# tonyckc/WT-PSE-code

Measured on AMD Instinct MI355X. Metric: training images/sec (256x256 fundus) — full WT-PSE iteration, higher is better.
Workload: dtype f32 (layers with > 16 output channels and the fused 1x1 heads: x2h (2 fp16 terms per fp32 operand — power-of-two operand scaling —, 3 fp16 MFMA products per multiply, fp32 accumulation); the 16-channel layers the same on 16x16x32, the 1-/3-channel input layers and small 1x1 convs fp32-input MFMA)

## Files before the change

### include/wtpse_hip.h

```cpp
#ifndef WTPSE_HIP_H
#define WTPSE_HIP_H
#ifdef __cplusplus
extern "C" {
#endif


int wtpse_pack_conv_weights(const float* params, const int* desc, int n_desc, float* packed, void* stream);

int wtpse_conv_fwd(const float* in0, int C0, const float* in1, int C1, const float* wpacked, const float* bias,
                   const float* pro0, const float* pro1, int pro_relu, float* out0, float* out1, int Csplit, float* stats,
                   int B, int H, int W, int Cout, int ksize, int relu_out, const float* mask_ref, unsigned* out_amax, void* stream);
int wtpse_conv_stats_blocks(int B, int H, int W);
int wtpse_conv_fwd_gram(const float* in0, int C0, const float* wpacked, const float* bias, const float* pro0, int pro_relu,
                        float* out0, float* gram_partial, int B, int H, int W, int Cout, int relu_out, unsigned* out_amax,
                        void* stream);

int wtpse_conv_x3_stats_blocks(int B, int H, int W, int Cout, int ksize);
int wtpse_x3r_enable(int on);
int wtpse_x3_xcd(int on);
int wtpse_x3_small_wide(int on);
int wtpse_x3_terms(int terms);
int wtpse_amax(const float* x, long long n, unsigned* amax_table, void* stream);
int wtpse_pack_conv_weights_x3(const float* params, const int* desc, int n_desc, unsigned short* packed, void* stream);
int wtpse_conv_fwd_x3(const float* in0, int C0, const float* in1, int C1, const unsigned short* wpacked, const float* bias,
                      const float* pro0, const float* pro1, int pro_relu, float* out0, float* out1, int Csplit, float* stats,
                      int B, int H, int W, int Cout, int ksize, int relu_out, const float* mask_ref, const unsigned* in_amax,
                      const unsigned* in_amax1, unsigned* out_amax, void* stream);

int wtpse_conv16_x3(const float* in0, int C0, const unsigned short* wx16, const float* bias, const float* pro0, int pro_relu,
                    float* out0, float* stats, float* gram_partial, const float* mask_ref, const float* bn_ss,
                    const float* bn_mean, int bn_relu, int B, int H, int W, int Cout, int relu_out, int in_is_grad,
                    const unsigned* in_amax, unsigned* out_amax, void* stream);
int wtpse_pack_conv16_x3(const float* params, const int* desc, int n_desc, unsigned short* packed, void* stream);

int wtpse_dgrad_bnb(const float* dy, int C, const float* wpacked, float* out0, float* out1, int Csplit, const float* bn_y,
                    const float* bn_ss, const float* bn_mean, int bn_relu, int bn_c0, int bn_c1, float* stats, int B, int H, int W,
                    int Cout, int ksize, void* stream);
int wtpse_dgrad_x3_bnb(const float* dy, int C, const unsigned short* wpacked, float* out0, float* out1, int Csplit,
                       const float* bn_y, const float* bn_ss, const float* bn_mean, int bn_relu, int bn_c0, int bn_c1, float* stats,
                       int B, int H, int W, int Cout, int ksize, const unsigned* in_amax, void* stream);

int wtpse_conv_fwd_bnf(const float* in0, int C0, const float* in1, int C1, const void* wpacked, int layout, const float* bias,
                       const float* pro0, const float* pro1, int pro_relu, float* out0, float* stats, const float* gamma,
                       const float* beta, float* running_mean, float* running_var, long long* num_batches, float momentum, float eps,
                       float* scale_shift, float* save_mean, float* save_invstd, double* partial2, unsigned* tickets, int B, int H,
                       int W, int Cout, int ksize, const unsigned* in_amax0, const unsigned* in_amax1, unsigned* act_amax, void* stream);

int wtpse_bnb_tail_partial2(int nblk, int Cout);
int wtpse_bnb_tail_tickets(int nblk, int Cout);
int wtpse_dgrad_bnb_coef(const float* dy, int C, const void* wpacked, int layout, float* out0, float* out1, int Csplit,
                         const float* bn_y, const float* bn_ss, const float* bn_mean, int bn_relu, int bn_c0, int bn_c1,
                         float* stats, const float* gamma, const float* invstd, float* coef, float* dgamma, float* dbeta,
                         int accumulate, double* partial2, unsigned* tickets, int B, int H, int W, int Cout, int ksize,
                         const unsigned* in_amax, void* stream);
int wtpse_dgrad_bnb_coef_frozen(const float* dy, int C, const void* wpacked, int layout, float* out0, float* out1, int Csplit,
                                const float* bn_y, const float* bn_ss, const float* bn_mean, int bn_relu, int bn_c0, int bn_c1,
                                float* stats, const float* gamma, const float* invstd, float* coef, float* dgamma, float* dbeta,
                                float* dbias, int accumulate, double* partial2, unsigned* tickets, int B, int H, int W, int Cout,
                                int ksize, const unsigned* in_amax, void* stream);

int wtpse_conv_wgrad(const float* dy, const float* x0, int C0, const float* x1, int C1, const float* pro0,
                     const float* pro1, int pro_relu, float* slab, float* dbias_slab, int ksplit, float* dw, float* dbias, int accumulate, int B, int H,
                     int W, int Cout, int ksize, void* stream);
int wtpse_wgrad_ksplit(int B, int H, int W, int Cin, int Cout);
int wtpse_wgrad_x3_supported(int Cin, int Cout, int ksize, int C0);
int wtpse_wgrad_x3_ksplit(int B, int H, int W, int Cin, int Cout);
int wtpse_conv_wgrad_x3(const float* dy, const float* x0, int C0, const float* x1, int C1, const float* pro0,
                        const float* pro1, int pro_relu, float* slab, int ksplit, float* dw, int accumulate, int B, int H, int W,
                        int Cout, int ksize, void* stream);

int wtpse_wgrad_r_supported(int Cin, int Cout, int ksize, int C0, int W);
int wtpse_wgrad_r_slabs(int B, int H, int W, int Cin, int Cout);
int wtpse_conv_wgrad_r(const float* dy, const float* x0, int C0, const float* x1, int C1, const float* pro0,
                       const float* pro1, int pro_relu, float* slab, float* dbias_slab, int nslab, float* dw, float* dbias,
                       int accumulate, int B, int H, int W, int Cout, const unsigned* dy_amax, const unsigned* x_amax0,
                       const unsigned* x_amax1, void* stream);

int wtpse_conv_wgrad_r_bn(const float* g, const float* bn_y, const float* bn_coef, const float* x0, int C0, const float* x1,
                          int C1, const float* pro0, const float* pro1, int pro_relu, float* slab, int nslab, float* dw,
                          int accumulate, int B, int H, int W, int Cout, void* stream);

int wtpse_bn_finalize(const float* stats_partial, int nblk, int C, long long count, const float* gamma, const float* beta,
                      float* running_mean, float* running_var, long long* num_batches, float momentum, float eps,
                      float* scale_shift, float* save_mean, float* save_invstd, unsigned* act_amax, void* stream);
int wtpse_bn_finalize_blend(const float* stats_partial, int nblk, int C, long long count, const float* gamma, const float* beta,
                            const float* running_mean, const float* running_var, double w, float eps, double* acc, double acc_count,
                            float* scale_shift, double* moments, double* div, unsigned* act_amax, void* stream);
int wtpse_act_bound(const float* scale_shift, int C, const unsigned* raw_amax, unsigned* act_amax, void* stream);
int wtpse_bn_eval_coeffs(const float* gamma, const float* beta, const float* running_mean, const float* running_var,
                         float eps, int C, float* scale_shift, void* stream);
int wtpse_affine_act(const float* y, const float* scale_shift, int relu, float* z, int B, int C, int HW, void* stream);
int wtpse_bn_bwd(const float* dz, const float* y, const float* scale_shift, int relu, const float* gamma,
                 const float* save_mean, const float* save_invstd, float* partial, float* coef, float* dgamma,
                 float* dbeta, int accumulate, float* dy, int B, int C, int HW, unsigned* amax, void* stream);
int wtpse_bn_bwd_nsplit(int B, int C, int HW);
int wtpse_bn_bwd_reduce(const float* dz, const float* y, const float* scale_shift, int relu, const float* save_mean,
                        const float* save_invstd, float* partial, float* sums_local, int B, int C, int HW, void* stream);
int wtpse_bn_bwd_apply(const float* dz, const float* y, const float* scale_shift, int relu, const float* gamma,
                       const float* save_mean, const float* save_invstd, const float* sums_local, const float* sums_global,
                       long long count_global, float* coef, float* dgamma, float* dbeta, int accumulate, float* dy, int B,
                       int C, int HW, unsigned* amax, void* stream);
int wtpse_bn_bwd_from_stats(const float* g, const float* y, const float* stats_partial, int nblk, const float* gamma,
                            const float* save_mean, const float* save_invstd, float* coef, float* dgamma, float* dbeta,
                            int accumulate, float* dy, int B, int C, int HW, unsigned* amax, void* stream);

int wtpse_bn_bwd_finalize_coef(const float* stats_partial, int nblk, int C, long long count, const float* gamma,
                               const float* save_mean, const float* save_invstd, float* coef, float* dgamma, float* dbeta,
                               int accumulate, void* stream);
int wtpse_bn_bwd_apply_coef(const float* g, const float* y, const float* coef, float* dy, int B, int C, int HW, unsigned* amax, void* stream);

int wtpse_bn_eval_coeffs_stats(const float* gamma, const float* beta, const float* running_mean, const float* running_var,
                               float eps, int C, float* scale_shift, float* save_mean, float* save_invstd, void* stream);
int wtpse_bn_bwd_frozen(const float* dz, const float* y, const float* scale_shift, int relu, const float* gamma,
                        const float* mean, const float* invstd, float* partial, float* coef, float* dgamma, float* dbeta,
                        float* dbias, int accumulate, float* dy, int B, int C, int HW, unsigned* amax, void* stream);
int wtpse_bn_bwd_from_stats_frozen(const float* g, const float* stats_partial, int nblk, const float* gamma, const float* invstd,
                                   float* coef, float* dgamma, float* dbeta, float* dbias, int accumulate, float* dy, int B, int C,
                                   int HW, unsigned* amax, void* stream);
int wtpse_bn_bwd_finalize_coef_frozen(const float* stats_partial, int nblk, int C, const float* gamma, const float* invstd,
                                      float* coef, float* dgamma, float* dbeta, float* dbias, int accumulate, void* stream);
int wtpse_bn_bwd_scale_coef(const float* g, const float* coef, float* dy, int B, int C, int HW, unsigned* amax, void* stream);

int wtpse_wt_loss_fwd(const float* z, int B, int C, int HW, float eps, float margin, int domain_num, int per_domain,
                      float* partial, float* gram, float* v, float* offdiag, float* diag, double* rowval,
                      float* dmmd_dv, float* losses, void* stream);
int wtpse_wt_split(int B, int HW, int* chunk_out);
int wtpse_wt_loss_fwd_partials(const float* partial, int S, int B, int HW, float eps, float margin, int domain_num,
                               int per_domain, float* gram, float* v, float* offdiag, float* diag, double* rowval,
                               float* dmmd_dv, float* losses, void* stream);
int wtpse_wt_gram_fwd(const float* z, int B, int C, int HW, float eps, float* partial, float* gram, float* v, float* offdiag,
                      float* diag, void* stream);
int wtpse_wt_final(const float* offdiag, const float* diag, int B, int Bnorm, float margin, const double* rowval, int R,
                   float* losses, void* stream);
int wtpse_wt_loss_bwd(const float* z, int B, int C, int HW, float margin, int domain_num, int per_domain,
                      const float* gram, const float* offdiag, const float* diag, const float* dmmd_dv,
                      const float* g_off, const float* g_diag, const float* g_dom, float w_off, float w_diag, float w_dom,
                      float* Mws, float* dz, int accumulate, void* stream);
int wtpse_wt_combine(const float* losses, int nmaps, float den, int mode, float* out, void* stream);
int wtpse_mmd_fwd(const float* v, int domain_num, int per_domain, double* rowval, float* dmmd_dv, void* stream);

int wtpse_maxpool2_fwd(const float* x, const float* pro, int relu, float* out, int B, int C, int H, int W, void* stream);
int wtpse_maxpool2_bwd(const float* x, const float* pro, int relu, const float* dout, float* dx, int accumulate, int B,
                       int C, int H, int W, void* stream);
int wtpse_maxpool2_bwd_stats_blocks(int B, int H, int W);
int wtpse_maxpool2_bwd_bnb(const float* x, const float* pro, int relu, const float* dout, float* dx, int accumulate,
                           const float* mean, float* stats, int B, int C, int H, int W, void* stream);
int wtpse_upsample2x_fwd(const float* x, const float* pro, int relu, float* out, int B, int C, int H, int W, void* stream);
int wtpse_upsample2x_bwd(const float* dout, float* dx, int accumulate, int B, int C, int H, int W, unsigned* amax, void* stream);
int wtpse_upsample2x_bwd_bn(const float* g, const float* bn_y, const float* bn_coef, float* dx, int B, int C, int H, int W,
                            unsigned* amax, void* stream);
int wtpse_upsample2x_fwd_stats(const float* x, float* out, float* stats, int B, int C, int H, int W, void* stream);
int wtpse_upsample2x_stats_blocks(int B, int H, int W);

int wtpse_resize_bilinear(const float* x, float* out, int B, int C, int H, int W, int Ho, int Wo, void* stream);

int wtpse_attn_fuse_fwd(const float* z, const float* wb, const float* emb, float coef, float* att, float* att_pre,
                        float* mask, float* fuse, int B, int CE, int HW, void* stream);
int wtpse_attn_fuse_bwd(const float* dfuse, const float* z, const float* emb, const float* att, const float* wb, float coef,
                        float* demb, float* dz, float* partial, float* d_wb, int accumulate, int B, int CE, int HW,
                        void* stream);

int wtpse_reparam_fwd(const float* mu, const float* logvar, const float* eps, float* z, long long n, void* stream);
int wtpse_reparam_bwd(const float* dz, const float* logvar, const float* eps, float* dlogvar, long long n, void* stream);
int wtpse_exp_half(const float* logvar, float* std_, long long n, void* stream);
int wtpse_reparam_student(const float* mu, const float* std_, const float* eps, float* z, long long n, void* stream);
int wtpse_nan_scrub(float* x, long long n, int* flag, void* stream);
int wtpse_randn(float* out, long long n, unsigned long long seed, unsigned long long offset,
                const unsigned long long* offset_dev, void* stream);
int wtpse_counter_add(void* counter, long long inc, int is64, void* stream);

int wtpse_reduce_blocks(long long n);
int wtpse_bce_sigmoid_fwd(const float* x, const float* t, long long n, float* partial, float* loss, void* stream);
int wtpse_bce_sigmoid_bwd(const float* x, const float* t, const float* g, float w, long long n, float* dx, void* stream);
int wtpse_pos_weight(const float* mask, const float* t, long long n, float* partial, float* sums, float* pw, void* stream);
int wtpse_pos_weight_from_sums(const float* sums, float* pw, void* stream);
int wtpse_bce_logits_pw_fwd(const float* x, const float* mask, const float* t, const float* pw, long long n, float* partial,
                            float* loss, void* stream);
int wtpse_bce_logits_pw_bwd(const float* x, const float* mask, const float* t, const float* pw, const float* g, float w,
                            long long n, float* dx, void* stream);
int wtpse_mse_fwd(const float* a, const float* b, long long n, float* partial, float* loss, void* stream);
int wtpse_mse_bwd(const float* a, const float* b, const float* g, float w, long long n, float* da, void* stream);
int wtpse_roi(const float* image, const float* logit, float* roi, float* od_pred, int B, int C, int HW, void* stream);
int wtpse_adam(float* p, const float* g, float* m, float* v, long long n, double lr, double beta1, double beta2, double eps,
               int step, const int* step_dev, void* stream);
int wtpse_adam_dev(float* p, const float* g, float* m, float* v, long long n, const float* lr_dev, double beta1, double beta2,
                   double eps, int step, const int* step_dev, const int* hold, void* stream);
int wtpse_adam_index(float* p, const float* g, float* m, float* v, const int* idx, int n_idx, const float* lr_dev, double beta1,
                     double beta2, double eps, int step, const int* step_dev, const int* hold, void* stream);
int wtpse_loss_log(const float* s0, const float* s1, const float* s2, const float* s3, const float* s4, const float* s5,
                   double* acc, int check_n, int* flag, const int* step_dev, void* stream);

int wtpse_signed_distance_ws(int B, int h, int w);
int wtpse_signed_distance(const float* t, float* phi, int* d2_out, int* d2_in, void* ws, int B, int h, int w, void* stream);
int wtpse_boundary_loss(const float* x, const float* mask, const float* phi, const float* alpha_dev, long long n, float* partial,
                        float* loss, float* dx, void* stream);

int wtpse_overlap_loss_ws(int B, int hw);
int wtpse_overlap_loss(const float* x, const float* mask, const float* t, const float* w_dev, int B, int hw, float fp, float fn,
                       float focal, float smooth, void* ws, float* plane_loss, float* loss, float* dx, void* stream);

int wtpse_entropy_loss_ws(int B, int hw);
int wtpse_entropy_loss(const float* x, const float* mask, int B, int hw, double margin, int reweight, void* ws, float* planes,
                       int* selected, float* loss, float* dx, void* stream);

int wtpse_lovasz_loss_ws(int B, int hw);
int wtpse_lovasz_loss(const float* x, const float* mask, const float* t, const float* w_dev, int B, int hw, void* ws,
                      float* plane_loss, int* ranks, float* loss, float* dx, void* stream);

int wtpse_avg_step(float* a0, const float* p0, long long n0, float* a1, const float* p1, long long n1, float* a2, const float* p2,
                   long long n2, float* a3, const float* p3, long long n3, int* count, const int* gate, const int* hold, void* stream);
int wtpse_avg_merge(float* acc, const float* seg, long long n, long long n_acc, long long n_seg, void* stream);

int wtpse_head_fwd(const float* x, const float* pro, int pro_relu, const float* w1, const float* b1, const float* w2,
                   const float* b2, const float* w3, const float* b3, int nc, float* h1, float* h2, float* y,
                   const unsigned* x_amax, int B, int HW, void* stream);
int wtpse_head_bwd(const float* dy, const float* x, const float* pro, int pro_relu, const float* h1, const float* h2,
                   const float* w1, const float* b1, const float* w2, const float* w3, int nc, float* dx, float* slab,
                   float* dparams, int accumulate, const unsigned* x_amax, const unsigned* dy_amax, int B, int HW, void* stream);
int wtpse_head_slabs(int B, int HW);

int wtpse_resample_u8(const unsigned char* in, unsigned char* out, const int* bounds, const int* kk, const int* tab, int ksize,
                      int N, int Hin, int Win, int C, int L, int vertical, void* stream);
int wtpse_input_finish(const unsigned char* img, const unsigned char* od, const int* xidx, const int* yidx, float* image,
                       float* od_out, float* oc_out, int N, int S, void* stream);
int wtpse_image_finish(const unsigned char* img, float* image, int N, int S, void* stream);

int wtpse_uniform_f64(double* out, long long n, unsigned long long seed, unsigned long long pos, void* stream);
int wtpse_aug_blur(const double* src, double* dst, const double* w, const int* src_index, int radius, int planes, int S, int axis,
                   int pre, double post, void* stream);
// ... 88 lines not shown
```

### wt-pse-code_amd/algorithms.py

```python
import torch
import torch.nn as nn

from wtpse_hip import nn as E
from wtpse_hip import ops

__all__ = ["get_algorithm_class", "WT_PSE", "compute_MMD"]


def get_algorithm_class(algorithm_name):
    if algorithm_name not in globals():
        raise NotImplementedError("Algorithm not found: {}".format(algorithm_name))
    return globals()[algorithm_name]


class compute_MMD(object):

    def __init__(self, domain_num, batch_size):
        self.domain_num = domain_num
        self.batch_size = batch_size
        self.kernel_type = "gaussian"

    def forward(self, inputs, **kwargs):
        v = inputs.contiguous()
        R = self.domain_num * self.batch_size
# ... 218 lines not shown
        ins_off, ins_diag, dom = _WtLossFn.apply(z, self.number_source_domain, self.per_domain_batch, float(self.margin), self.eps)
        return ins_off + ins_diag, dom

    def _as_input(self, t):
        if not t.is_cuda:
            raise RuntimeError("WT_PSE on MI355X takes device tensors (got %s)" % t.device)
        return t.detach().to(torch.float32).contiguous()

    def _get_anchor(self):
        a = self.__dict__.get("_anchor")
        if a is None or a.device != self._flat.device:
            a = torch.zeros(1, device=self._flat.device, requires_grad=True)
            object.__setattr__(self, "_anchor", a)
        return a

    def _embedding(self, inputs, training, tape):
        want = tape is not None
        x1, c_inc = E.convd_fwd(self.inc, inputs, training, want)
        feat, c_unet = E.unet_fwd(self, x1, training, want)
        emb, c_mu = E.head_fwd(self.mu, feat, (0, 2), want)
        if want:
            tape.inc, tape.unet, tape.mu = c_inc, c_unet, c_mu
        return emb

    def _forward_update(self, inputs, mask, wt_in, want_tape):
        with ops.fwd_scope(inputs.device):
            return self._forward_update_body(inputs, mask, wt_in, want_tape)

    def _forward_update_body(self, inputs, mask, wt_in, want_tape):
        hp = self.hparams
        t = E.Tape()
        t.shape_prior = bool(hp['shape_prior'])
        training = self.training
        if not t.shape_prior:
            emb = self._embedding(inputs, training, t if want_tape else None)
            out, _ = E._conv(self.outc[0], emb)
            t.emb = emb
            return (out,), t
        coef = float(hp['shape_attention_coeffient'])
        D, n = self.number_source_domain, self.per_domain_batch

        def prior_chain():
            w = E.deepwt_fwd(self.wt_model, wt_in, want_tape, want_gram=not (self._dp is not None and self._dp.exact))
            th = E.teacher_fwd(self.prior_dist, E.Act(w.z2, None, True), mask, training, True, want_tape)
            eps = self.next_noise(th.mu.shape)
            z_post = ops.reparam_fwd(th.mu, th.logvar, eps)
            losses = torch.empty((2, 3), dtype=torch.float32, device=inputs.device)
            st1 = self._wt_loss(w.z1, D, n, losses[0], w.g1)
            st2 = self._wt_loss(w.z2, D, n, losses[1], w.g2)
            return w, th, eps, z_post, st1, st2, ops.wt_combine(losses, 3.0, 0)

        second = None if (self._dp is not None and self._dp.exact) else E.second_stream(inputs.device)
        if second is not None:
            main = torch.cuda.current_stream()
            E.stream_wait(second, main)
            with torch.cuda.stream(second):
                w, th, eps, z_post, st1, st2, scal = prior_chain()
        emb = self._embedding(inputs, training, t if want_tape else None)
        if second is None:
            w, th, eps, z_post, st1, st2, scal = prior_chain()
        else:
            E.stream_wait(main, second)
            z_post.record_stream(main)
            scal.record_stream(main)
        att, _, att_mask, fuse = ops.attn_fuse_fwd(z_post, self.attention_layer.layer1.weight.data_ptr(), emb, coef,
                                                   True, False, True)
        fuse_in = self._outc_input(fuse, z_post)
        out, _ = E._conv(self.outc[0], fuse_in)
        if want_tape:
            t.w, t.th, t.eps, t.z_post, t.att, t.emb, t.fuse, t.st1, t.st2, t.coef = w, th, eps, z_post, att, emb, fuse_in, st1, st2, coef
        return (out, att_mask, scal), t

    def _wt_loss(self, z, D, n, losses_out, gram=None):
        if self._dp is not None and self._dp.exact:
            return self._dp.wt_loss_fwd(z, D, n, float(self.margin), self.eps, losses_out)
        return ops.wt_loss_fwd(z, D, n, float(self.margin), self.eps, losses_out, gram)

    def _wt_loss_bwd(self, st, dz, mask_in=False, **kw):
        acc = 3 if mask_in else 1
        if self._dp is not None:
            return self._dp.wt_loss_bwd(st, dz, acc, **kw)
        return ops.wt_loss_bwd(st, dz, acc, **kw)

    def _backward_update(self, t, d_out, d_ins=None, d_dom=None, w_ins=1.0, w_dom=1.0):
        self.begin_backward()
        if d_out is None:
            d_out = ops.zero_(torch.empty((t.emb.shape[0], self.n_classes) + tuple(t.emb.shape[2:]), dtype=torch.float32, device=t.emb.device))
        d_out = d_out.contiguous()
        outc = self.outc[0]
        if not t.shape_prior:
            E._wgrad(outc, d_out, t.emb)
            demb, _ = E._dgrad(outc, d_out)
        else:
            E._wgrad(outc, d_out, t.fuse)
            dfuse, _ = E._dgrad(outc, d_out)
            dz_cat = None
            if self.cat_shape:
                dz_cat = dfuse[:, self.feature_dim:].contiguous()
                dfuse = dfuse[:, :self.feature_dim].contiguous()
            al = self.attention_layer.layer1
            d_wb = self.gview(al.weight)
            self.gview(al.bias)
            demb, dz_post = ops.attn_fuse_bwd(dfuse, t.z_post, t.emb, t.att, al.weight.data_ptr(), t.coef, d_wb.data_ptr(), True)
            if dz_cat is not None:
                ops.axpy(dz_post, dz_cat)
            gi = d_ins.contiguous() if d_ins is not None else None
            gd = d_dom.contiguous() if d_dom is not None else None
            kw = dict(g_off=gi, g_diag=gi, g_dom=gd, w_off=w_ins / 3.0, w_diag=w_ins / 3.0, w_dom=w_dom / 3.0)

            def prior_chain_bwd():
                dlogvar = ops.reparam_bwd(dz_post, t.th.logvar, t.eps)
                d_relu_z2 = E.teacher_bwd(self.prior_dist, t.th, dz_post, dlogvar)
                self.grads_ready(self.prior_dist)
                dz2 = d_relu_z2
                self._wt_loss_bwd(t.st2, dz2, mask_in=True, **kw)
                E.deepwt_bwd(self.wt_model, t.w, dz2, lambda dz1: self._wt_loss_bwd(t.st1, dz1, **kw))

            second = None if (self._dp is not None and self._dp.exact) else E.second_stream(dz_post.device)
            if second is not None:
                main = torch.cuda.current_stream()
                E.stream_wait(second, main)
                with torch.cuda.stream(second):
                    prior_chain_bwd()
                for g in (dz_post, gi, gd):
                    if g is not None:
                        g.record_stream(second)
                E.note_join(self, second)
            else:
                prior_chain_bwd()
        dfeat = E.head_bwd(self.mu, t.mu, demb, (0, 2))
        self.grads_ready(self.mu, self.attention_layer)
        dx1 = E.unet_bwd(self, t.unet, dfeat, decoder_done=lambda: self.grads_ready(self.up1, self.up4), below_x1=t.inc.c3)
        E.convd_bwd(self.inc, t.inc, dx1, need_dx=False)
        self.end_backward()
```

### wt-pse-code_amd/shape_networks.py

```python
import torch
import torch.nn as nn

from wtpse_hip import nn as E
from wtpse_hip import ops

__all__ = ["ShapeVariationalDist_x"]


class _ShapeUpdateFn(torch.autograd.Function):
    @staticmethod
    def forward(ctx, anchor, net, main_network, x, mask):
        scal, tape = net._forward_update(main_network, x, mask, want_tape=True)
        ctx.net, ctx.tape = net, tape
        return scal[0], scal[1], scal[2], scal[3], scal[4]

    @staticmethod
    def backward(ctx, d_kd, d_tot, d_off, d_diag, d_dom):
        g_off = d_tot if d_off is None else (d_off if d_tot is None else d_tot + d_off)
        g_diag = d_tot if d_diag is None else (d_diag if d_tot is None else d_tot + d_diag)
        ctx.net._backward_update(ctx.tape, d_kd, g_off, g_diag, d_dom,
                                 w_kd=0.0 if d_kd is None else 1.0, w_off=0.0 if g_off is None else 1.0,
                                 w_diag=0.0 if g_diag is None else 1.0, w_dom=0.0 if d_dom is None else 1.0)
        ctx.tape = None
        return None, None, None, None, None
# ... 40 lines not shown
        if tab is not None and x.data_ptr() == inputs.data_ptr():
            ops.amax_attach(x, tab)
        with ops.fwd_scope(x.device):
            mu, fmap = self._student_mu(E.Act(x), self.training, None, want_fmap=True)
        if not training:
            return mu
        logvar, _ = E.head_fwd(self.logvar_prior, fmap, (0, 2, 4), False)
        eps = self.next_noise(mu.shape)
        return ops.reparam_student(mu, logvar, eps, self._flag), mu

    def compute_whitening_loss(self, z):
        from algorithms import _WtLossFn
        return _WtLossFn.apply(z, 3, self.batch_size, float(self.margin), self.eps)

    def _as_input(self, t):
        if not t.is_cuda:
            raise RuntimeError("ShapeVariationalDist_x on MI355X takes device tensors (got %s)" % t.device)
        return t.detach().to(torch.float32).contiguous()

    def _get_anchor(self):
        a = self.__dict__.get("_anchor")
        if a is None or a.device != self._flat.device:
            a = torch.zeros(1, device=self._flat.device, requires_grad=True)
            object.__setattr__(self, "_anchor", a)
        return a

    def _student_mu(self, feat, training, tape, want_fmap=False):
        want = tape is not None
        fmap, c_unet = E.unet_fwd(self, feat, training, want)
        mu, c_mu = E.head_fwd(self.mu_prior, fmap, (0, 2, 4), want)
        ops.nan_scrub_(mu, self._flag)
        if want:
            tape.unet, tape.hmu = c_unet, c_mu
        return (mu, fmap) if want_fmap else mu

    def _forward_update(self, main_network, x, mask, want_tape):
        with ops.fwd_scope(x.device):
            return self._forward_update_body(main_network, x, mask, want_tape)

    def _forward_update_body(self, main_network, x, mask, want_tape):
        t = E.Tape()
        training = self.training
        def teacher():
            w1 = E.deepwt_fwd(main_network.wt_model, x, want_tape=False)
            th = E.teacher_fwd(main_network.prior_dist, E.Act(w1.z2, None, True), mask, main_network.training,
                               want_logvar=False, want_tape=False)
            return th.mu
        synced = main_network._dp is not None and main_network._dp.bn_sync
        side = None if synced else E.second_stream(x.device)
        if side is not None:
            main = torch.cuda.current_stream()
            E.stream_wait(side, main)
            with torch.cuda.stream(side):
                mu_t = teacher()
        else:
            mu_t = teacher()
        w2 = E.deepwt_fwd(self.wt_model, x, want_tape, want_gram=not (self._dp is not None and self._dp.exact))
        mu_s = self._student_mu(E.Act(w2.z2, None, True), training, t if want_tape else None)
        if side is not None:
            E.stream_wait(main, side)
            mu_t.record_stream(main)
        scal = torch.empty((5,), dtype=torch.float32, device=x.device)
        ops.mse_fwd(mu_t, mu_s, out=scal[0:1])
        losses = torch.empty((2, 3), dtype=torch.float32, device=x.device)
        n = self.batch_size
        st1 = self._wt_loss(w2.z1, 3, n, losses[0], w2.g1)
        st2 = self._wt_loss(w2.z2, 3, n, losses[1], w2.g2)
        ops.wt_combine(losses, 3.0, 1, out=scal[1:5])
        if want_tape:
            t.w2, t.mu_t, t.mu_s, t.st1, t.st2 = w2, mu_t, mu_s, st1, st2
        return scal, t

    def _wt_loss(self, z, D, n, losses_out, gram=None):
        if self._dp is not None and self._dp.exact:
            return self._dp.wt_loss_fwd(z, D, n, float(self.margin), self.eps, losses_out)
        return ops.wt_loss_fwd(z, D, n, float(self.margin), self.eps, losses_out, gram)

    def _wt_loss_bwd(self, st, dz, mask_in=False, **kw):
        acc = 3 if mask_in else 1
        if self._dp is not None:
            return self._dp.wt_loss_bwd(st, dz, acc, **kw)
        return ops.wt_loss_bwd(st, dz, acc, **kw)

    def _backward_update(self, t, g_kd=None, g_off=None, g_diag=None, g_dom=None, w_kd=1.0, w_off=1.0, w_diag=1.0, w_dom=1.0):
        self.begin_backward()
        c = lambda g: g.contiguous() if g is not None else None
        g_kd, g_off, g_diag, g_dom = c(g_kd), c(g_off), c(g_diag), c(g_dom)
        dmu = ops.mse_bwd(t.mu_s, t.mu_t, g_kd, w_kd)
        dfmap = E.head_bwd(self.mu_prior, t.hmu, dmu, (0, 2, 4))
        d_relu_z2 = E.unet_bwd(self, t.unet, dfmap, decoder_done=lambda: self.grads_ready(self.up1, self.logvar_prior))
        dz2 = d_relu_z2
        self._wt_loss_bwd(t.st2, dz2, mask_in=True, g_off=g_off, g_diag=g_diag, g_dom=g_dom, w_off=w_off / 3.0, w_diag=2.0 * w_diag / 3.0,
                          w_dom=w_dom / 3.0)
        E.deepwt_bwd(self.wt_model, t.w2, dz2,
                     lambda dz1: self._wt_loss_bwd(t.st1, dz1, g_off=g_off, g_diag=g_diag, g_dom=g_dom, w_off=w_off / 3.0,
                                                   w_diag=0.0, w_dom=w_dom / 3.0))
        self.end_backward()
```

### wt-pse-code_amd/wtpse_hip/csrc/conv.hip

```cpp
#include "internal.h"

#define WTPSE_P16_KC(KS) ((KS) == 3 ? 4 : 8)

struct ConvArgs {
  const float* in0;
  const float* in1;
  const float* wp;
  const float* bias;
  const float* pro0;
  const float* pro1;
  float* out0;
  float* out1;
  float* stats;
  const float* mask;
  const unsigned* in_amax;
  float in_scale;
  unsigned* out_amax;
  float* gram;
  const float* bn_ss;
  const float* bn_mean;
  int bn_c0, bn_c1, bn_relu;
  BnbTail tail;
  BnfTail ftail;
  int B, H, W;
  int C0, C1, Cin, CinP;
  int Cout, CoutP, Csplit;
  int pro_relu;
  int relu_out;
  int tiles_x, tiles_y;
  int xcd_tiles;
};


template <bool P16> struct AccT { typedef f32x16 type; };
template <> struct AccT<true> { typedef f32x4 type; };
__device__ __forceinline__ f32x4 mfma(float a, float b, f32x4 c) { return mfma16(a, b, c); }
__device__ __forceinline__ f32x16 mfma(float a, float b, f32x16 c) { return mfma32(a, b, c); }

template <int PE>
struct PlaneStride {
  static constexpr int value = ((PE - 16 + 31) / 32) * 32 + 16;
};

template <int KS, int MODE, int TWL, bool DB, int EPI>
__global__ __launch_bounds__(256, 3) void conv_fwd_k(ConvArgs a) {
  constexpr bool MASK = EPI == 1, BNB = EPI == 2;
  constexpr int TAPS = KS * KS, PAD = KS / 2;
  constexpr int TW = 1 << TWL, TH = 256 / TW;
  constexpr int PITCH = TW + 2 * PAD, ROWS = TH + 2 * PAD;
  constexpr int PE = PITCH * ROWS;
  constexpr int NPOS = (PE + 255) / 256;
  constexpr int S = PlaneStride<NPOS * 256>::value;
  constexpr bool XP = (MODE == 3 || MODE == 4);
  constexpr int XT = MODE == 4 ? 2 : 3;
  constexpr bool P16 = (MODE == 0) || XP;
  static_assert(!XP || KS == 3, "MODE 3 / 4 is the 3x3 path");
  constexpr int MT = P16 ? 1 : MODE;
  constexpr int MB = P16 ? 16 : 32;
  constexpr int CB = MB * MT;
  constexpr int NT = P16 ? 4 : 2;
  constexpr int NB = P16 ? 16 : 32;
  constexpr int KC = P16 ? WTPSE_P16_KC(KS) : 8;
  constexpr int KQ = P16 ? 4 : 2;
  constexpr int NACC = P16 ? 4 : 16;
  constexpr int CB4 = CB / 4;
  constexpr int NW = (KC * TAPS * CB4 + 255) / 256;
  constexpr int PEP = (PE + 7) & ~7;
  constexpr int XS_SZ = XP ? 2 * XT * PEP * 4 : KC * S;
  constexpr int WS_SZ = XP ? 0 : NW * 1024;
  constexpr int GRAM_SZ = (P16 && KS == 3) ? 4 * 16 * 65 + 4 * 256 : 0;
  constexpr int RED_SZ = 4 * CB * 2 > GRAM_SZ ? 4 * CB * 2 : GRAM_SZ;
  constexpr int MAIN_SZ = (XS_SZ + WS_SZ) > RED_SZ ? (XS_SZ + WS_SZ) : RED_SZ;
  __shared__ __attribute__((aligned(16))) float smem[MAIN_SZ + CB + (BNB ? 4 * CB : 0)];
  float* bias_s = smem + MAIN_SZ;
  const float* bnp_s = bias_s + CB;
  float* Xs = smem;
  float* Ws = smem + XS_SZ;

  const int tid = threadIdx.x, lane = tid & 63, wave = tid >> 6;
  int tile = (int)blockIdx.x, cblk = (int)blockIdx.y;
  if (a.xcd_tiles > 0) {
    const int L = (int)(blockIdx.y * gridDim.x + blockIdx.x), sl = L >> 3;
    cblk = sl % (int)gridDim.y;
    tile = (L & 7) * a.xcd_tiles + sl / (int)gridDim.y;
  }
  int bx = tile;
  const int tx = bx % a.tiles_x;
  bx /= a.tiles_x;
  const int ty = bx % a.tiles_y;
  const int b = bx / a.tiles_y;
  const int cout0 = cblk * CB;
  const int HW = a.H * a.W;
  if (tid < CB) bias_s[tid] = (a.bias && cout0 + tid < a.Cout) ? a.bias[cout0 + tid] : 0.f;
  if (BNB && tid < CB) bnb_stage<CB>(bias_s + CB + tid, cout0 + tid, a);

  int off[NT];
#pragma unroll
  for (int nt = 0; nt < NT; ++nt) {
    int p = wave * 64 + nt * NB + (lane & (NB - 1));
    off[nt] = (p >> TWL) * PITCH + (p & (TW - 1));
  }

  typename AccT<P16>::type acc[MT][NT];
#pragma unroll
  for (int mt = 0; mt < MT; ++mt)
#pragma unroll
    for (int nt = 0; nt < NT; ++nt)
#pragma unroll
      for (int r = 0; r < NACC; ++r) acc[mt][nt][r] = 0.f;

  if constexpr (XP) {
    u32x4* Xq = reinterpret_cast<u32x4*>(smem);
    const int g4 = lane >> 4;
    constexpr int PB = (PE + 63) / 64, NIT = (2 * PB + 3) / 4;
    const __amdgpu_buffer_rsrc_t rs0 = make_rsrc(a.in0 + (size_t)b * a.C0 * HW, (unsigned)a.C0 * HW * 4u);
    const bool any_pro = MODE == 4 || a.pro0 != nullptr || a.pro_relu != 0;
    const unsigned sx_raw = MODE == 4 ? amax_load(a.in_amax) : 0u;
    __builtin_amdgcn_sched_barrier(0);
    float xv[NIT][8];
    int ipos[NIT], ihalf[NIT];
    bool iin[NIT];
    float psc[2][8], psh[2][8];
#pragma unroll
    for (int hh = 0; hh < 2; ++hh)
#pragma unroll
      for (int j = 0; j < 8; ++j) {
        const int cg = min(hh * 8 + j, a.C0 - 1);
        psc[hh][j] = a.pro0 ? a.pro0[2 * cg] : 1.f;
        psh[hh][j] = a.pro0 ? a.pro0[2 * cg + 1] : 0.f;
      }
#pragma unroll
    for (int i = 0; i < NIT; ++i) {
      const int blk = __builtin_amdgcn_readfirstlane(i * 4 + wave);
      ihalf[i] = blk >= PB ? 1 : 0;
      const int p = (blk - ihalf[i] * PB) * 64 + lane;
      ipos[i] = (blk < 2 * PB && p < PE) ? p : -1;
      const int r = p / PITCH, x = p - r * PITCH;
      const int gy = ty * TH + r - PAD, gx = tx * TW + x - PAD;
      iin[i] = ipos[i] >= 0 && gy >= 0 && gy < a.H && gx >= 0 && gx < a.W;
// ... 133 lines not shown
      const int cmax = (first ? a.C0 : a.C1) - 1;
#pragma unroll
      for (int c = 0; c < KC; ++c) {
        const int cg = min(cbase + c, cmax);
        const float sc = pro ? pro[2 * cg] : 1.f, sh = pro ? pro[2 * cg + 1] : 0.f;
#pragma unroll
        for (int i = 0; i < NPOS; ++i) {
          float v = fmaf(xv[c][i], sc, sh);
          if (relu) v = fmaxf(v, 0.f);
          xv[c][i] = gpos[i] >= 0 ? v : 0.f;
        }
      }
    }
#pragma unroll
    for (int c = 0; c < KC; ++c)
#pragma unroll
      for (int i = 0; i < NPOS; ++i) Xs[c * S + tid + 256 * i] = xv[c][i];
#pragma unroll
    for (int it = 0; it < NW; ++it) *reinterpret_cast<f32x4*>(Ws + (tid + 256 * it) * 4) = wv[it];
  };
  if (DB) issue_loads(0);
  for (int c0 = 0; c0 < a.CinP; c0 += KC) {
    const int kc = min(KC, a.CinP - c0);
    __syncthreads();
    if (!DB) issue_loads(c0);
    stash(c0);
    __syncthreads();
    if (DB && c0 + KC < a.CinP) issue_loads(c0 + KC);
    const int nq = kc / KQ;
    for (int q = 0; q < nq; ++q) {
      const int cl = q * KQ + (lane / NB);
      const float* xrow = Xs + cl * S;
      const float* wrow = Ws + cl * TAPS * CB + (lane & (MB - 1));
      float av[TAPS][MT], bv[TAPS][NT];
#pragma unroll
      for (int t = 0; t < TAPS; ++t) {
        const int toff = (t / KS) * PITCH + (t % KS);
#pragma unroll
        for (int mt = 0; mt < MT; ++mt) av[t][mt] = wrow[t * CB + mt * MB];
#pragma unroll
        for (int nt = 0; nt < NT; ++nt) bv[t][nt] = xrow[off[nt] + toff];
      }
#pragma unroll
      for (int t = 0; t < TAPS; ++t)
#pragma unroll
        for (int nt = 0; nt < NT; ++nt)
#pragma unroll
          for (int mt = 0; mt < MT; ++mt) acc[mt][nt] = mfma(av[t][mt], bv[t][nt], acc[mt][nt]);
    }
  }
  }
  if (a.bias) {
    float bz[MT][NACC];
#pragma unroll
    for (int mt = 0; mt < MT; ++mt)
#pragma unroll
      for (int r = 0; r < NACC; ++r)
        bz[mt][r] = bias_s[P16 ? ((lane >> 4) * 4 + r) : (mt * 32 + (r & 3) + 8 * (r >> 2) + 4 * (lane >> 5))];
#pragma unroll
    for (int mt = 0; mt < MT; ++mt)
#pragma unroll
      for (int r = 0; r < NACC; ++r)
#pragma unroll
        for (int nt = 0; nt < NT; ++nt) acc[mt][nt][r] += bz[mt][r];
  }

  const bool want_stats = a.stats != nullptr;
  if (want_stats) __syncthreads();
  float* red = smem;
  const int C1out = a.Cout - a.Csplit;
  int poff[NT];
#pragma unroll
  for (int nt = 0; nt < NT; ++nt) {
    int p = wave * 64 + nt * NB + (lane & (NB - 1));
    int gy = ty * TH + (p >> TWL), gx = tx * TW + (p & (TW - 1));
    poff[nt] = (gy < a.H && gx < a.W) ? gy * a.W + gx : -1;
  }
  const __amdgpu_buffer_rsrc_t rs_o0 = make_rsrc(a.out0 + (size_t)b * a.Csplit * HW, (unsigned)a.Csplit * HW * 4u);
  const __amdgpu_buffer_rsrc_t rs_o1 = a.out1 ? make_rsrc(a.out1 + (size_t)b * C1out * HW, (unsigned)C1out * HW * 4u) : rs_o0;
  const int Cbn = a.bn_c1 - a.bn_c0;
  const __amdgpu_buffer_rsrc_t rs_m = MASK ? make_rsrc(a.mask + (size_t)b * a.Cout * HW, (unsigned)a.Cout * HW * 4u)
                                      : BNB ? make_rsrc(a.mask + (size_t)b * Cbn * HW, (unsigned)Cbn * HW * 4u) : rs_o0;
  const int clane = P16 ? (lane >> 4) * 4 : (lane >> 5) * 4;
  unsigned pvo[NT];
#pragma unroll
  for (int nt = 0; nt < NT; ++nt) pvo[nt] = poff[nt] >= 0 ? (unsigned)(clane * HW + poff[nt]) * 4u : BUF_OOB;
  constexpr int NSV = NACC * 2;
  const bool full = ty * TH + TH <= a.H && tx * TW + TW <= a.W && cout0 + CB <= a.Cout;
  if (!full) {
#pragma unroll
    for (int mt = 0; mt < MT; ++mt)
#pragma unroll
      for (int r = 0; r < NACC; ++r) {
        const bool cvalid = cout0 + (P16 ? r : (mt * 32 + (r & 3) + 8 * (r >> 2))) + clane < a.Cout;
#pragma unroll
        for (int nt = 0; nt < NT; ++nt) acc[mt][nt][r] = (cvalid && poff[nt] >= 0) ? acc[mt][nt][r] : 0.f;
      }
  }
  if (a.relu_out) {
#pragma unroll
    for (int mt = 0; mt < MT; ++mt)
#pragma unroll
      for (int nt = 0; nt < NT; ++nt)
#pragma unroll
        for (int r = 0; r < NACC; ++r) acc[mt][nt][r] = out_clamp<EPI>(acc[mt][nt][r], 0.f);
  }
  if constexpr (P16 && KS == 3) {
    if (a.gram) {
      __syncthreads();
      float* zs = smem + wave * (16 * 65);
#pragma unroll
      for (int nt = 0; nt < NT; ++nt)
#pragma unroll
        for (int r = 0; r < NACC; ++r) zs[((lane >> 4) * 4 + r) * 65 + nt * 16 + (lane & 15)] = acc[0][nt][r];
      __builtin_amdgcn_wave_barrier();
      f32x4 g = {0.f, 0.f, 0.f, 0.f};
#pragma unroll
      for (int st = 0; st < 16; ++st) {
        const float v = zs[(lane & 15) * 65 + 4 * st + (lane >> 4)];
        g = mfma16(v, v, g);
      }
      float* gs = smem + 4 * 16 * 65 + wave * 256;
#pragma unroll
      for (int r = 0; r < 4; ++r) gs[((lane >> 4) * 4 + r) * 16 + (lane & 15)] = g[r];
      __syncthreads();
      const float* g0 = smem + 4 * 16 * 65;
      a.gram[(size_t)tile * 256 + tid] = g0[tid] + g0[256 + tid] + g0[512 + tid] + g0[768 + tid];
      __syncthreads();
    }
  }
  if constexpr (EPI == 0) {
    if (a.out_amax) {
      unsigned am = 0u;
#pragma unroll
      for (int mt = 0; mt < MT; ++mt)
#pragma unroll
        for (int nt = 0; nt < NT; ++nt)
#pragma unroll
          for (int r = 0; r < NACC; ++r) am = max(am, amax_bits(acc[mt][nt][r]));
      amax_publish_wave(a.out_amax, am, (unsigned)tile * 4u + (unsigned)wave);
    }
  }
  const unsigned hw4 = (unsigned)HW * 4u;
  const bool defer = want_stats && (BNB ? a.tail.tickets != nullptr : a.ftail.tickets != nullptr);
#pragma unroll
  for (int mt = 0; mt < MT; ++mt) {
    float mk[NACC][NT];
    if (MASK) {
#pragma unroll
      for (int r = 0; r < NACC; ++r) {
        const int cbase = cout0 + (P16 ? r : (mt * 32 + (r & 3) + 8 * (r >> 2)));
#pragma unroll
        for (int nt = 0; nt < NT; ++nt) mk[r][nt] = buf_load(rs_m, pvo[nt], (unsigned)min(cbase, a.Cout) * hw4);
      }
    }
    if (BNB) {
#pragma unroll
      for (int r = 0; r < NACC; ++r) {
        const int cbase = cout0 + (P16 ? r : (mt * 32 + (r & 3) + 8 * (r >> 2)));
        const bool bn = cbase >= a.bn_c0 && cbase < a.bn_c1;
        const unsigned soff = (unsigned)(bn ? cbase - a.bn_c0 : 0) * hw4;
#pragma unroll
        for (int nt = 0; nt < NT; ++nt) mk[r][nt] = buf_load(rs_m, bn ? pvo[nt] : BUF_OOB, soff);
      }
    }
    float bmu[NACC];
#pragma unroll
    for (int r = 0; r < NACC; ++r) {
      const int cbase = cout0 + (P16 ? r : (mt * 32 + (r & 3) + 8 * (r >> 2)));
      const bool second = a.out1 != nullptr && cbase >= a.Csplit;
      const __amdgpu_buffer_rsrc_t rs_o = second ? rs_o1 : rs_o0;
      const unsigned soff = (unsigned)(second ? min(cbase, a.Cout) - a.Csplit : min(cbase, a.Csplit)) * hw4;
      float bsc = 0.f, bsh = 1.f;
      bmu[r] = 0.f;
      if (BNB) {
        const int crel = (P16 ? r : (mt * 32 + (r & 3) + 8 * (r >> 2))) + clane;
        bsc = bnp_s[crel];
        bsh = bnp_s[CB + crel];
        bmu[r] = bnp_s[2 * CB + crel];
      }
#pragma unroll
      for (int nt = 0; nt < NT; ++nt) {
        float v = acc[mt][nt][r];
        if (MASK && !(mk[r][nt] > 0.f)) v = 0.f;
        if (BNB) {
          if (!bn_relu_live_opaque(mk[r][nt], bsc, bsh)) v = 0.f;
          acc[mt][nt][r] = v;
        }
        if (!defer) buf_store(rs_o, pvo[nt], soff, v);
      }
    }
    if (want_stats) {
      float sv[NSV];
#pragma unroll
      for (int r = 0; r < NACC; ++r) {
        float s1 = 0.f, s2 = 0.f;
#pragma unroll
        for (int nt = 0; nt < NT; ++nt) {
#pragma clang fp contract(off)
          if (BNB) {
            const float v = acc[mt][nt][r];
            s1 += v;
            s2 += v * (mk[r][nt] - bmu[r]);
          } else {
            const float v = acc[mt][nt][r];
            s1 += v;
            s2 += v * v;
          }
        }
        sv[r * 2 + 0] = s1;
        sv[r * 2 + 1] = s2;
      }
      constexpr int LB = P16 ? 4 : 5;
      constexpr int HB = P16 ? 3 : 5;
#pragma unroll
      for (int st = 0; st < HB; ++st) {
        const int half = NSV >> (st + 1);
        const bool up = (lane >> st) & 1;
#pragma unroll
        for (int i = 0; i < NSV / 2; ++i) {
          if (i < half) {
            float keep = up ? sv[i + half] : sv[i];
            float send = up ? sv[i] : sv[i + half];
            sv[i] = keep + __shfl_xor(send, 1 << st, 64);
          }
        }
      }
#pragma unroll
      for (int st = HB; st < LB; ++st) sv[0] += __shfl_xor(sv[0], 1 << st, 64);
      int idx = 0;
#pragma unroll
      for (int st = 0; st < HB; ++st) idx += ((lane >> st) & 1) * (NSV >> (st + 1));
      const int k = idx & 1, rr = idx >> 1;
      const int crel = P16 ? ((lane >> 4) * 4 + rr) : (mt * 32 + (rr & 3) + 8 * (rr >> 2) + 4 * (lane >> 5));
      if (((lane & (NB - 1)) >> HB) == 0) red[(wave * CB + crel) * 2 + k] = sv[0];
    }
  }
  if (want_stats) {
    __syncthreads();
    if (tid < CB * 2) {
      int crel = tid >> 1;
      const float s = red[tid] + red[CB * 2 + tid] + red[2 * CB * 2 + tid] + red[3 * CB * 2 + tid];
      if (BNB) {
        const int c = cout0 + crel;
        if (c >= a.bn_c0 && c < a.bn_c1) pub_store(a.stats + ((size_t)tile * Cbn + c - a.bn_c0) * 2 + (tid & 1), s);
      } else if (cout0 + crel < a.Cout) {
        pub_store(a.stats + ((size_t)tile * a.Cout + cout0 + crel) * 2 + (tid & 1), s);
      }
    }
  }
  TailTicket tk;
  tk.old = 0u;
  tk.armed = 0;
  if (defer) {
    if constexpr (BNB) tk = bnb_tail_begin<CB>(a.tail, a.bn_c0, a.bn_c1, cout0, tile, cblk, tid);
    else tk = bnf_tail_begin(a.ftail, tile, cblk, tid);
  }
  if (defer) {
#pragma unroll
    for (int mt = 0; mt < MT; ++mt)
#pragma unroll
      for (int r = 0; r < NACC; ++r) {
        const int cbase = cout0 + (P16 ? r : (mt * 32 + (r & 3) + 8 * (r >> 2)));
        const bool second = a.out1 != nullptr && cbase >= a.Csplit;
        const __amdgpu_buffer_rsrc_t rs_o = second ? rs_o1 : rs_o0;
        const unsigned soff = (unsigned)(second ? min(cbase, a.Cout) - a.Csplit : min(cbase, a.Csplit)) * hw4;
#pragma unroll
        for (int nt = 0; nt < NT; ++nt) buf_store(rs_o, pvo[nt], soff, acc[mt][nt][r]);
      }
    if constexpr (BNB)
      bnb_tail<CB>(tk, a.tail, a.stats, a.bn_mean, a.bn_c0, a.bn_c1, cout0, tile, cblk, tid,
                   reinterpret_cast<double*>(red), reinterpret_cast<int*>(red + 520));
    else
      bnf_tail<CB>(tk, a.ftail, a.stats, a.Cout, cout0, tile, cblk, tid, reinterpret_cast<double*>(red),
                   reinterpret_cast<int*>(red + 520));
  }
}

template <int KS, int MODE, bool DB, int EPI>
static int launch_fwd(const ConvArgs& a, hipStream_t st) {
  constexpr int CB = (MODE == 0 || MODE == 3 || MODE == 4) ? 16 : 32 * MODE;
  ConvArgs args = a;
  const Tiling t = conv_tiling(a.B, a.H, a.W);
  args.tiles_x = t.tiles_x;
  args.tiles_y = t.tiles_y;
  dim3 grid((unsigned)t.tiles, (unsigned)ceil_div(a.CoutP, CB));
  static const bool xcd_on = [] { const char* e = getenv("WTPSE_C16_XCD"); return !(e && e[0] == '0'); }();
  args.xcd_tiles = (xcd_on && grid.x % 8 == 0 && (long long)grid.x * grid.y >= 64) ? (int)(grid.x / 8) : 0;
  const bool in_launch = tail_in_launch((long long)grid.x * grid.y);
  if (!in_launch) args.tail.tickets = args.ftail.tickets = nullptr;
  if (args.tail.tickets) bnb_tail_geometry(args.tail, (int)grid.x, a.Cout, (double)a.B * a.H * a.W);
  if (args.ftail.tickets) bnf_tail_geometry(args.ftail, (int)grid.x, a.Cout, (double)a.B * a.H * a.W);
  if (t.TW == 16)
    hipLaunchKernelGGL((conv_fwd_k<KS, MODE, 4, DB, EPI>), grid, dim3(256), 0, st, args);
  else
    hipLaunchKernelGGL((conv_fwd_k<KS, MODE, 5, DB, EPI>), grid, dim3(256), 0, st, args);
  const int rc = wtpse_status();
  return rc == 0 && !in_launch ? tail_after_launch(a, (int)grid.x, st) : rc;
}

extern "C" int wtpse_conv_stats_blocks(int B, int H, int W) { return conv_tiling(B, H, W).tiles; }

static int conv_check(const ConvCall& c, int layout) {
  const BnbArgs& bn = c.bn;
  const BnbTail& t = c.tail;
  const BnfTail& f = c.ftail;
  const bool bnb = bn.mean != nullptr;
  WTPSE_REQUIRE(layout == CONV_FP32 || layout == CONV_X3 || layout == CONV_C16);
  WTPSE_REQUIRE(c.in0 && c.w && c.out0 && c.B > 0 && c.H > 0 && c.W > 0 && c.C0 > 0 && c.C1 >= 0 && c.Cout > 0);
  WTPSE_REQUIRE(c.ksize == 1 || c.ksize == 3);
  WTPSE_REQUIRE((c.C1 == 0) == (c.in1 == nullptr));
  WTPSE_REQUIRE(c.Csplit > 0 && c.Csplit <= c.Cout && ((c.Csplit == c.Cout) == (c.out1 == nullptr)));
  WTPSE_REQUIRE(c.Csplit == c.Cout || c.Csplit % 16 == 0);
  WTPSE_REQUIRE(!(c.stats && c.relu_out));
  WTPSE_REQUIRE(bnb || !(c.stats && c.mask_ref));
  WTPSE_REQUIRE(bnb || !(c.mask_ref && c.out1));
  WTPSE_REQUIRE(!bnb || (c.mask_ref && c.stats && bn.ss && !c.bias && !c.relu_out && !c.gram && bn.c0 >= 0 && bn.c0 < bn.c1 &&
                         bn.c1 <= c.Cout && bn.c0 % 16 == 0 && (bn.c1 % 16 == 0 || bn.c1 == c.Cout)));
  WTPSE_REQUIRE(c.C1 == 0 || c.C0 % 16 == 0);
  WTPSE_REQUIRE(!(c.out_amax && (c.mask_ref || bnb)));
  WTPSE_REQUIRE(!c.gram || (c.Cout == 16 && !c.relu_out));
  WTPSE_REQUIRE(!t.tickets || (bnb && t.partial2 && t.gamma && t.invstd && t.coef && t.dgamma && t.dbeta));
  WTPSE_REQUIRE(!f.tickets || (!bnb && c.stats && !c.gram && f.partial2 && f.gamma && f.beta && f.scale_shift && f.save_mean &&
                               f.save_invstd && (f.rmean == nullptr) == (f.rvar == nullptr)));
  if (layout == CONV_X3) {
    const X3Tiling g = x3_tiling(c.B, c.H, c.W, c.Cout, c.ksize);
    WTPSE_REQUIRE(!c.gram && !(c.in_amax1 && !c.in1) && ((c.C0 + c.C1 + 15) & ~15) <= (g.mt == 2 && !g.half ? 512 : 256));
  }
  if (layout == CONV_C16)
    WTPSE_REQUIRE(c.ksize == 3 && c.C0 <= 16 && c.Cout <= 16 && (((uintptr_t)c.w) & 15) == 0 && !c.in1 && !c.pro1);
  return 0;
}

static int conv_launch_fwd(const ConvCall& c, bool c16, hipStream_t st) {
  const bool bnb = c.bn.mean != nullptr;
  ConvArgs a;
  a.tail = c.tail;
  a.ftail = c.ftail;
  a.bn_ss = c.bn.ss; a.bn_mean = c.bn.mean; a.bn_relu = c.bn.relu; a.bn_c0 = bnb ? c.bn.c0 : 0; a.bn_c1 = bnb ? c.bn.c1 : 0;
  a.in0 = c.in0; a.in1 = c.in1; a.wp = static_cast<const float*>(c.w); a.bias = c.bias; a.pro0 = c.pro0; a.pro1 = c.pro1;
  a.out0 = c.out0; a.out1 = c.out1; a.stats = c.stats; a.mask = c.mask_ref; a.gram = c.gram;
  a.in_amax = c16 ? c.in_amax0 : nullptr; a.in_scale = c16 ? X3_FWD_SCALE : 1.f; a.out_amax = c.out_amax;
  a.B = c.B; a.H = c.H; a.W = c.W; a.C0 = c.C0; a.C1 = c.C1; a.Cin = c.C0 + c.C1; a.CinP = c16 ? 16 : (a.Cin + 3) & ~3;
  a.Cout = c.Cout; a.CoutP = (c.Cout + 15) & ~15; a.Csplit = c.Csplit; a.pro_relu = c.pro_relu; a.relu_out = c.relu_out;
  a.tiles_x = a.tiles_y = 0;
#define FWD(KS, M, DB) (bnb ? launch_fwd<KS, M, DB, 2>(a, st) : c.mask_ref ? launch_fwd<KS, M, DB, 1>(a, st) : launch_fwd<KS, M, DB, 0>(a, st))
  if (c16) return (g_x3_terms == 2 && (!c.in_is_grad || c.in_amax0)) ? FWD(3, 4, false) : FWD(3, 3, false);
  int mode = c.Cout <= 16 ? 0 : (c.Cout % 64 == 0 ? 2 : 1);
  const int tiles = conv_tiling(c.B, c.H, c.W).tiles;
  if (mode == 2 && tiles * (a.CoutP / 64) < 512) mode = 1;
  if (mode == 1 && tiles * ceil_div(a.CoutP, 32) < 384) mode = 0;
  const int cb = mode == 0 ? 16 : 32 * mode;
  const bool db = tiles * ceil_div(a.CoutP, cb) < 768 && a.CinP > (mode == 0 ? WTPSE_P16_KC(c.ksize) : 8);
#define FWD_DB(KS, M) (db ? FWD(KS, M, true) : FWD(KS, M, false))
  if (c.ksize == 3) return mode == 0 ? FWD_DB(3, 0) : mode == 1 ? FWD_DB(3, 1) : FWD_DB(3, 2);
  return mode == 0 ? FWD_DB(1, 0) : mode == 1 ? FWD_DB(1, 1) : FWD_DB(1, 2);
#undef FWD_DB
#undef FWD
}

int conv_run(const ConvCall& c, int layout, hipStream_t st) {
  if (const int rc = conv_check(c, layout)) return rc;
  return layout == CONV_X3 ? conv_launch_x3(c, st) : conv_launch_fwd(c, layout == CONV_C16, st);
}

extern "C" int wtpse_conv_fwd(const float* in0, int C0, const float* in1, int C1, const float* wpacked,
                              const float* bias, const float* pro0, const float* pro1, int pro_relu, float* out0, float* out1,
                              int Csplit, float* stats, int B, int H, int W, int Cout, int ksize, int relu_out,
                              const float* mask_ref, unsigned* out_amax, void* stream) {
  ConvCall c;
  c.in0 = in0; c.C0 = C0; c.in1 = in1; c.C1 = C1; c.w = wpacked; c.bias = bias; c.pro0 = pro0; c.pro1 = pro1; c.pro_relu = pro_relu;
  c.out0 = out0; c.out1 = out1; c.Csplit = Csplit; c.stats = stats; c.mask_ref = mask_ref; c.out_amax = out_amax;
  c.B = B; c.H = H; c.W = W; c.Cout = Cout; c.ksize = ksize; c.relu_out = relu_out;
  return conv_run(c, CONV_FP32, (hipStream_t)stream);
}

extern "C" int wtpse_dgrad_bnb(const float* dy, int C, const float* wpacked, float* out0, float* out1, int Csplit,
                               const float* bn_y, const float* bn_ss, const float* bn_mean, int bn_relu, int bn_c0, int bn_c1,
                               float* stats, int B, int H, int W, int Cout, int ksize, void* stream) {
  WTPSE_REQUIRE(bn_y && bn_ss && bn_mean && stats);
  ConvCall c;
  c.in0 = dy; c.C0 = C; c.w = wpacked; c.out0 = out0; c.out1 = out1; c.Csplit = Csplit; c.stats = stats; c.mask_ref = bn_y;
  c.bn.ss = bn_ss; c.bn.mean = bn_mean; c.bn.relu = bn_relu; c.bn.c0 = bn_c0; c.bn.c1 = bn_c1;
  c.B = B; c.H = H; c.W = W; c.Cout = Cout; c.ksize = ksize;
  return conv_run(c, CONV_FP32, (hipStream_t)stream);
}

extern "C" int wtpse_conv16_x3(const float* in0, int C0, const unsigned short* wx16, const float* bias, const float* pro0,
                               int pro_relu, float* out0, float* stats, float* gram_partial, const float* mask_ref,
                               const float* bn_ss, const float* bn_mean, int bn_relu, int B, int H, int W, int Cout, int relu_out,
                               int in_is_grad, const unsigned* in_amax, unsigned* out_amax, void* stream) {
  ConvCall c;
  c.in0 = in0; c.C0 = C0; c.w = wx16; c.bias = bias; c.pro0 = pro0; c.pro_relu = pro_relu; c.out0 = out0; c.Csplit = Cout;
  c.stats = stats; c.gram = gram_partial; c.mask_ref = mask_ref; c.in_amax0 = in_amax; c.in_is_grad = in_is_grad; c.out_amax = out_amax;
  c.bn.ss = bn_ss; c.bn.mean = bn_mean; c.bn.relu = bn_relu; c.bn.c1 = Cout;
  c.B = B; c.H = H; c.W = W; c.Cout = Cout; c.ksize = 3; c.relu_out = relu_out;
  return conv_run(c, CONV_C16, (hipStream_t)stream);
}

extern "C" int wtpse_conv_fwd_bnf(const float* in0, int C0, const float* in1, int C1, const void* wpacked, int layout,
                                  const float* bias, const float* pro0, const float* pro1, int pro_relu, float* out0, float* stats,
                                  const float* gamma, const float* beta, float* running_mean, float* running_var,
                                  long long* num_batches, float momentum, float eps, float* scale_shift, float* save_mean,
                                  float* save_invstd, double* partial2, unsigned* tickets, int B, int H, int W, int Cout, int ksize,
                                  const unsigned* in_amax0, const unsigned* in_amax1, unsigned* act_amax, void* stream) {
  WTPSE_REQUIRE(stats && gamma && beta && scale_shift && save_mean && save_invstd && partial2 && tickets);
  ConvCall c;
  c.in0 = in0; c.C0 = C0; c.in1 = in1; c.C1 = C1; c.w = wpacked; c.bias = bias; c.pro0 = pro0; c.pro1 = pro1; c.pro_relu = pro_relu;
  c.out0 = out0; c.Csplit = Cout; c.stats = stats; c.in_amax0 = in_amax0; c.in_amax1 = in_amax1;
  BnfTail& t = c.ftail;
  t.partial2 = partial2; t.tickets = tickets; t.gamma = gamma; t.beta = beta; t.rmean = running_mean; t.rvar = running_var;
  t.nbt = num_batches; t.momentum = momentum; t.eps = eps; t.scale_shift = scale_shift; t.save_mean = save_mean;
  t.save_invstd = save_invstd; t.act_amax = act_amax;
  c.B = B; c.H = H; c.W = W; c.Cout = Cout; c.ksize = ksize;
  return conv_run(c, layout, (hipStream_t)stream);
}

extern "C" int wtpse_bnb_tail_partial2(int nblk, int Cout) { return bnb_tail_groups(nblk) * bnb_tail_ctot(Cout) * 2; }
extern "C" int wtpse_bnb_tail_tickets(int nblk, int Cout) { return bnb_tail_t2off(nblk, Cout) + (Cout + 15) / 16; }

static int dgrad_bnb_coef(ConvCall c, int layout, void* stream) {
  const BnbTail& t = c.tail;
  WTPSE_REQUIRE(c.mask_ref && c.bn.ss && c.bn.mean && c.stats && t.gamma && t.invstd && t.coef && t.dgamma && t.dbeta && t.partial2 &&
                t.tickets);
  c.in_is_grad = 1;
  return conv_run(c, layout, (hipStream_t)stream);
}

extern "C" int wtpse_dgrad_bnb_coef(const float* dy, int C, const void* wpacked, int layout, float* out0, float* out1, int Csplit,
                                    const float* bn_y, const float* bn_ss, const float* bn_mean, int bn_relu, int bn_c0, int bn_c1,
                                    float* stats, const float* gamma, const float* invstd, float* coef, float* dgamma,
                                    float* dbeta, int accumulate, double* partial2, unsigned* tickets, int B, int H, int W,
                                    int Cout, int ksize, const unsigned* in_amax, void* stream) {
  ConvCall c;
  c.in0 = dy; c.C0 = C; c.w = wpacked; c.out0 = out0; c.out1 = out1; c.Csplit = Csplit; c.stats = stats; c.mask_ref = bn_y;
  c.bn.ss = bn_ss; c.bn.mean = bn_mean; c.bn.relu = bn_relu; c.bn.c0 = bn_c0; c.bn.c1 = bn_c1; c.in_amax0 = in_amax;
  BnbTail& t = c.tail;
  t.partial2 = partial2; t.tickets = tickets; t.gamma = gamma; t.invstd = invstd; t.coef = coef; t.dgamma = dgamma; t.dbeta = dbeta;
  t.accumulate = accumulate;
  c.B = B; c.H = H; c.W = W; c.Cout = Cout; c.ksize = ksize;
  return dgrad_bnb_coef(c, layout, stream);
}

extern "C" int wtpse_dgrad_bnb_coef_frozen(const float* dy, int C, const void* wpacked, int layout, float* out0, float* out1,
                                           int Csplit, const float* bn_y, const float* bn_ss, const float* bn_mean, int bn_relu,
                                           int bn_c0, int bn_c1, float* stats, const float* gamma, const float* invstd, float* coef,
                                           float* dgamma, float* dbeta, float* dbias, int accumulate, double* partial2,
                                           unsigned* tickets, int B, int H, int W, int Cout, int ksize, const unsigned* in_amax,
                                           void* stream) {
  WTPSE_REQUIRE(dbias);
  ConvCall c;
  c.in0 = dy; c.C0 = C; c.w = wpacked; c.out0 = out0; c.out1 = out1; c.Csplit = Csplit; c.stats = stats; c.mask_ref = bn_y;
  c.bn.ss = bn_ss; c.bn.mean = bn_mean; c.bn.relu = bn_relu; c.bn.c0 = bn_c0; c.bn.c1 = bn_c1; c.in_amax0 = in_amax;
  BnbTail& t = c.tail;
  t.partial2 = partial2; t.tickets = tickets; t.gamma = gamma; t.invstd = invstd; t.coef = coef; t.dgamma = dgamma; t.dbeta = dbeta;
  t.dbias = dbias; t.accumulate = accumulate;
  c.B = B; c.H = H; c.W = W; c.Cout = Cout; c.ksize = ksize;
  return dgrad_bnb_coef(c, layout, stream);
}

__global__ __launch_bounds__(256) void pack_weights_x3p16_k(const float* __restrict__ params, const int* __restrict__ desc,
                                                            unsigned short* __restrict__ packed) {
  const int* d = desc + blockIdx.y * 8;
  const int w_off = d[0], Co = d[1], Ci = d[2];
  const float* w = params + w_off;
  __shared__ float red[4];
  float m = 0.f;
  for (int e = threadIdx.x; e < Co * Ci * 9; e += 256) m = fmaxf(m, fabsf(w[e]));
  for (int o = 32; o > 0; o >>= 1) m = fmaxf(m, __shfl_xor(m, o, 64));
  if ((threadIdx.x & 63) == 0) red[threadIdx.x >> 6] = m;
  __syncthreads();
  m = fmaxf(fmaxf(red[0], red[1]), fmaxf(red[2], red[3]));
  const float sc = x3_scale_from_amax(__builtin_bit_cast(unsigned, m));
  for (int dir = 0; dir < 2; ++dir) {
    const int base = d[4 + dir];
    if (base < 0) continue;
    const int R = dir == 0 ? Co : Ci, K = dir == 0 ? Ci : Co;
    if (blockIdx.x == 0 && threadIdx.x == 0) {
      float* hdr = reinterpret_cast<float*>(packed + base);
// ... 441 lines not shown
```

### wt-pse-code_amd/wtpse_hip/csrc/internal.h

```cpp
#pragma once
#include <cstdlib>
#include "common.h"

#define WTPSE_INTERNAL __attribute__((visibility("hidden")))

WTPSE_INTERNAL extern int g_x3_terms;

struct BnbArgs {
  const float* ss = nullptr;
  const float* mean = nullptr;
  int relu = 0, c0 = 0, c1 = 0;
};
struct ConvCall {
  const float* in0 = nullptr; int C0 = 0;
  const float* in1 = nullptr; int C1 = 0;
  const void* w = nullptr;
  const float* bias = nullptr;
  const float* pro0 = nullptr; const float* pro1 = nullptr; int pro_relu = 0;
  float* out0 = nullptr; float* out1 = nullptr; int Csplit = 0;
  float* stats = nullptr;
  const float* mask_ref = nullptr;
  float* gram = nullptr;
  const unsigned* in_amax0 = nullptr; const unsigned* in_amax1 = nullptr;
  int in_is_grad = 0;
  unsigned* out_amax = nullptr;
  BnbArgs bn;
  BnbTail tail = bnb_tail_none();
  BnfTail ftail = bnf_tail_none();
  int B = 0, H = 0, W = 0, Cout = 0, ksize = 0, relu_out = 0;
};
enum { CONV_FP32 = 0, CONV_X3 = 1, CONV_C16 = 2 };
WTPSE_INTERNAL int conv_run(const ConvCall& c, int layout, hipStream_t st);
WTPSE_INTERNAL int conv_launch_x3(const ConvCall& c, hipStream_t st);

struct Tiling {
  int TW, TH, tiles_x, tiles_y, tiles;
};
static inline Tiling make_tiling(int B, int H, int W, bool narrow, int pixels) {
  Tiling t;
  t.TW = narrow ? 16 : 32; t.TH = pixels / t.TW;
  t.tiles_x = ceil_div(W, t.TW); t.tiles_y = ceil_div(H, t.TH); t.tiles = B * t.tiles_x * t.tiles_y;
  return t;
}
static inline Tiling conv_tiling(int B, int H, int W, int pixels = 256) { return make_tiling(B, H, W, W <= 16, pixels); }
struct X3Tiling {
  int mt;
  int px;
  int half;
  int small;
  Tiling t;
};
WTPSE_INTERNAL X3Tiling x3_tiling(int B, int H, int W, int Cout, int ksize);

struct WgradCall {
  const float* dy = nullptr;
  const float* x0 = nullptr; int C0 = 0;
  const float* x1 = nullptr; int C1 = 0;
  const float* pro0 = nullptr; const float* pro1 = nullptr; int pro_relu = 0;
  float* slab = nullptr; float* dbias_slab = nullptr; int nslab = 0;
  float* dw = nullptr; float* dbias = nullptr; int accumulate = 0;
  const float* bn_y = nullptr; const float* bn_coef = nullptr; const unsigned* dy_amax = nullptr;
  const unsigned* x_amax0 = nullptr; const unsigned* x_amax1 = nullptr;
  int B = 0, H = 0, W = 0, Cout = 0, ksize = 0;
};
enum { WGRAD_FP32 = 0, WGRAD_X3 = 1, WGRAD_R = 2 };
WTPSE_INTERNAL int wgrad_run(const WgradCall& c, int family, hipStream_t st);
WTPSE_INTERNAL int wgrad_launch_x3(const WgradCall& c, hipStream_t st);
WTPSE_INTERNAL int wgrad_launch_r(const WgradCall& c, hipStream_t st);

struct WgradX3Geometry {
  Tiling t;
  int q, blk, nci, nx, ksplit;
};
WTPSE_INTERNAL WgradX3Geometry wgrad_x3_geometry(int B, int H, int W, int Cin, int Cout);
struct WgradRPlan {
  int mf, nf, nw, pairs, nci, wpp, nseg, rseg, units, strips, nslab;
};
WTPSE_INTERNAL bool wgrad_r_plan(int B, int H, int W, int Cin, int Cout, WgradRPlan& p);

static inline bool tail_in_launch(long long workgroups) {
  static const long long max_wgs = [] { const char* e = getenv("WTPSE_TAIL_MAX_WGS"); return e ? atoll(e) : 8192ll; }();
  return workgroups <= max_wgs;
}
template <class Args>
static inline int tail_after_launch(const Args& a, int nblk, hipStream_t stream) {
  const BnbTail& tl = a.tail;
  const BnfTail& fl = a.ftail;
  const long long count = (long long)a.B * a.H * a.W;
  if (tl.tickets && tl.dbias)
    return wtpse_bn_bwd_finalize_coef_frozen(a.stats, nblk, a.bn_c1 - a.bn_c0, tl.gamma, tl.invstd, tl.coef, tl.dgamma, tl.dbeta,
                                             tl.dbias, tl.accumulate, stream);
  if (tl.tickets)
    return wtpse_bn_bwd_finalize_coef(a.stats, nblk, a.bn_c1 - a.bn_c0, count, tl.gamma, a.bn_mean, tl.invstd, tl.coef, tl.dgamma,
                                      tl.dbeta, tl.accumulate, stream);
  if (fl.tickets)
    return wtpse_bn_finalize(a.stats, nblk, a.Cout, count, fl.gamma, fl.beta, fl.rmean, fl.rvar, fl.nbt, fl.momentum, fl.eps,
                             fl.scale_shift, fl.save_mean, fl.save_invstd, fl.act_amax, stream);
  return 0;
}
```

### wt-pse-code_amd/wtpse_hip/csrc/pointwise.hip

```cpp
#include "common.h"

__device__ __forceinline__ float act_in(float v, const float* pro, int c, int relu) {
  if (pro) v = fmaf(v, pro[2 * c], pro[2 * c + 1]);
  return relu ? fmaxf(v, 0.f) : v;
}

__device__ __forceinline__ float block_sum(float v, float* sh4) {
  v = wave_xor_sum(v, 32);
  __syncthreads();
  if ((threadIdx.x & 63) == 0) sh4[threadIdx.x >> 6] = v;
  __syncthreads();
  return sh4[0] + sh4[1] + sh4[2] + sh4[3];
}

__global__ __launch_bounds__(256) void maxpool2_fwd_k(const float* __restrict__ x, const float* __restrict__ pro, int relu,
                                                      float* __restrict__ out, int C, int H, int W, long long total) {
  const int Ho = H / 2, Wo = W / 2;
  long long i = (long long)blockIdx.x * 256 + threadIdx.x;
  if (i >= total) return;
  int xo = (int)(i % Wo);
  long long r = i / Wo;
  int yo = (int)(r % Ho);
  long long bc = r / Ho;
  int c = (int)(bc % C);
// ... 276 lines not shown
        for (int t = 0; t < 10; ++t) w[t] = bn_dy(k1, k2, k3, w[t], v[t]);
        if (xb == 0) w[0] = 0.f;
        if (2 * xb + 8 >= Wo) w[9] = 0.f;
      }
#pragma unroll
      for (int e = 0; e < 4; ++e) {
        const int xx = xb + e;
        float rowsum = 0.f;
#pragma unroll
        for (int dxo = -1; dxo <= 2; ++dxo) {
          const int xo = 2 * xx + dxo;
          if (xo < 0 || xo >= Wo) continue;
          rowsum += up_w(xo, W, xx) * w[2 * e + dxo + 1];
        }
        g[e] += wy * rowsum;
      }
    }
    float* dst = dx + (size_t)bc * H * W + (size_t)yy * W + xb;
    float4 o = make_float4(g[0], g[1], g[2], g[3]);
    if (accumulate) {
      const float4 p = *reinterpret_cast<const float4*>(dst);
      o = make_float4(p.x + o.x, p.y + o.y, p.z + o.z, p.w + o.w);
    }
    *reinterpret_cast<float4*>(dst) = o;
    am = max(am, max(max(amax_bits(o.x), amax_bits(o.y)), max(amax_bits(o.z), amax_bits(o.w))));
  }
  if (amax) amax_publish_wave(amax, am, (blockIdx.x + blockIdx.y * gridDim.x) * 4u + (threadIdx.x >> 6));
}

__global__ __launch_bounds__(256) void resize_bilinear_k(const float* __restrict__ x, float* __restrict__ out, int H, int W,
                                                         int Ho, int Wo, float sy, float sx, long long total) {
  long long i = (long long)blockIdx.x * 256 + threadIdx.x;
  if (i >= total) return;
  int xo = (int)(i % Wo);
  long long r = i / Wo;
  int yo = (int)(r % Ho);
  long long bc = r / Ho;
  float fy = sy * (yo + 0.5f) - 0.5f, fx = sx * (xo + 0.5f) - 0.5f;
  if (fy < 0.f) fy = 0.f;
  if (fx < 0.f) fx = 0.f;
  int y0 = (int)fy, x0 = (int)fx;
  int y1 = y0 + (y0 < H - 1 ? 1 : 0), x1 = x0 + (x0 < W - 1 ? 1 : 0);
  float ly = fy - (float)y0, lx = fx - (float)x0;
  const float* src = x + (size_t)bc * H * W;
  float v00 = src[y0 * W + x0], v01 = src[y0 * W + x1], v10 = src[y1 * W + x0], v11 = src[y1 * W + x1];
  out[i] = (1.f - ly) * ((1.f - lx) * v00 + lx * v01) + ly * ((1.f - lx) * v10 + lx * v11);
}

__global__ __launch_bounds__(256) void relu_mask_k(const float* __restrict__ dz, const float* __restrict__ ref,
                                                   float* __restrict__ dy, int accumulate, long long n) {
  long long i = (long long)blockIdx.x * 256 + threadIdx.x;
  if (i >= n) return;
  float g = ref[i] > 0.f ? dz[i] : 0.f;
  dy[i] = accumulate ? dy[i] + g : g;
}

__global__ __launch_bounds__(256) void axpy_k(float* __restrict__ dst, const float* __restrict__ src, float alpha, long long n) {
  long long i = (long long)blockIdx.x * 256 + threadIdx.x;
  if (i < n) dst[i] = fmaf(alpha, src[i], dst[i]);
}

__global__ __launch_bounds__(256) void relu_mask_v_k(const float4* __restrict__ dz, const float4* __restrict__ ref,
                                                     float4* __restrict__ dy, int accumulate, long long n4) {
  long long i = (long long)blockIdx.x * 256 + threadIdx.x;
  if (i >= n4) return;
  const float4 d = dz[i], r = ref[i];
  float4 g = make_float4(r.x > 0.f ? d.x : 0.f, r.y > 0.f ? d.y : 0.f, r.z > 0.f ? d.z : 0.f, r.w > 0.f ? d.w : 0.f);
  if (accumulate) {
    const float4 o = dy[i];
    g.x += o.x; g.y += o.y; g.z += o.z; g.w += o.w;
  }
  dy[i] = g;
}

__global__ __launch_bounds__(256) void axpy_v_k(float4* __restrict__ dst, const float4* __restrict__ src, float alpha, long long n4) {
  long long i = (long long)blockIdx.x * 256 + threadIdx.x;
  if (i >= n4) return;
  const float4 s4 = src[i];
  float4 d = dst[i];
  d.x = fmaf(alpha, s4.x, d.x); d.y = fmaf(alpha, s4.y, d.y); d.z = fmaf(alpha, s4.z, d.z); d.w = fmaf(alpha, s4.w, d.w);
  dst[i] = d;
}

__global__ __launch_bounds__(256) void reduce_rows_k(const float* __restrict__ partial, int rows, int cols,
                                                     float* __restrict__ out, int accumulate, float scale) {
  int j = blockIdx.x * 256 + threadIdx.x;
  if (j >= cols) return;
  double s = 0.0;
  for (int r = 0; r < rows; ++r) s += partial[(size_t)r * cols + j];
  float v = (float)s * scale;
  out[j] = accumulate ? out[j] + v : v;
}

__global__ __launch_bounds__(256) void reduce_rows_tall_k(const float* __restrict__ partial, int rows, int cols,
                                                          float* __restrict__ out, int accumulate, float scale) {
  __shared__ double sh[256];
  const int j = blockIdx.x, t = threadIdx.x;
  double s = 0.0;
  for (int r = t; r < rows; r += 256) s += partial[(size_t)r * cols + j];
  sh[t] = s;
  __syncthreads();
  for (int m = 128; m >= 1; m >>= 1) {
    if (t < m) sh[t] += sh[t + m];
    __syncthreads();
  }
  if (t == 0) {
    float v = (float)sh[0] * scale;
    out[j] = accumulate ? out[j] + v : v;
  }
}

__global__ __launch_bounds__(256) void attn_fuse_fwd_k(const float* __restrict__ z, const float* __restrict__ wb,
                                                       const float* __restrict__ emb, float coef, float* __restrict__ att,
                                                       float* __restrict__ att_pre, float* __restrict__ mask,
                                                       float* __restrict__ fuse, int CE, int HW, long long total) {
  long long i = (long long)blockIdx.x * 256 + threadIdx.x;
  if (i >= total) return;
  long long b = i / HW;
  int p = (int)(i - b * HW);
  float pre = fmaf(wb[0], z[i], wb[1]);
  float a = sigmoidf_(pre);
  if (att) att[i] = a;
  if (att_pre) att_pre[i] = pre;
  if (mask) mask[i] = a > 0.75f ? 1.f : 0.f;
  for (int c = 0; c < CE; ++c) {
    size_t idx = ((size_t)b * CE + c) * HW + p;
    float e = emb[idx];
    fuse[idx] = coef * e + a * e;
  }
}

__global__ __launch_bounds__(256) void attn_fuse_bwd_k(const float* __restrict__ dfuse, const float* __restrict__ z,
                                                       const float* __restrict__ emb, const float* __restrict__ att,
                                                       const float* __restrict__ wb, float coef, float* __restrict__ demb,
                                                       float* __restrict__ dz, float* __restrict__ partial, int CE, int HW,
                                                       long long total) {
  __shared__ float sh[4];
  long long i = (long long)blockIdx.x * 256 + threadIdx.x;
  float dw = 0.f, db = 0.f;
  if (i < total) {
    long long b = i / HW;
    int p = (int)(i - b * HW);
    float a = att[i];
    float datt = 0.f;
    for (int c = 0; c < CE; ++c) {
      size_t idx = ((size_t)b * CE + c) * HW + p;
      float g = dfuse[idx];
      datt = fmaf(g, emb[idx], datt);
      demb[idx] = g * (coef + a);
    }
    float dpre = datt * a * (1.f - a);
    if (dz) dz[i] = dpre * wb[0];
    dw = dpre * z[i];
    db = dpre;
  }
  dw = block_sum(dw, sh);
  db = block_sum(db, sh);
  if (threadIdx.x == 0) {
    partial[(size_t)blockIdx.x * 2] = dw;
    partial[(size_t)blockIdx.x * 2 + 1] = db;
  }
}

__global__ __launch_bounds__(256) void reparam_fwd_k(const float* __restrict__ mu, const float* __restrict__ logvar,
                                                     const float* __restrict__ eps, float* __restrict__ z, long long n) {
  long long i = (long long)blockIdx.x * 256 + threadIdx.x;
// ... 302 lines not shown
  if (W % 4 == 0 && (((uintptr_t)dout | (uintptr_t)dx) & 15) == 0) {
    hipLaunchKernelGGL(upsample2x_bwd_v_k<false>, up_bwd_grid(H * (W / 4), B * C, amax != nullptr), dim3(256), 0, ST, dout, dx, accumulate,
                       B * C, H, W, nullptr, nullptr, C, amax);
    return wtpse_status();
  }
  hipLaunchKernelGGL(upsample2x_bwd_k, GRID1(total), dim3(256), 0, ST, dout, dx, accumulate, H, W, total);
  const int rc = wtpse_status();
  return (rc || !amax) ? rc : wtpse_amax(dx, total, amax, stream);
}
extern "C" int wtpse_upsample2x_bwd_bn(const float* g, const float* bn_y, const float* bn_coef, float* dx, int B, int C, int H, int W,
                                       unsigned* amax, void* stream) {
  WTPSE_REQUIRE(g && bn_y && bn_coef && dx && B > 0 && C > 0 && H > 0 && W > 0 && W % 4 == 0);
  WTPSE_REQUIRE((((uintptr_t)g | (uintptr_t)bn_y | (uintptr_t)dx) & 15) == 0);
  hipLaunchKernelGGL(upsample2x_bwd_v_k<true>, up_bwd_grid(H * (W / 4), B * C, amax != nullptr), dim3(256), 0, ST, g, dx, 0, B * C, H, W,
                     bn_y, bn_coef, C, amax);
  return wtpse_status();
}
extern "C" int wtpse_resize_bilinear(const float* x, float* out, int B, int C, int H, int W, int Ho, int Wo, void* stream) {
  WTPSE_REQUIRE(x && out && B > 0 && C > 0 && H > 0 && W > 0 && Ho > 0 && Wo > 0);
  long long total = (long long)B * C * Ho * Wo;
  hipLaunchKernelGGL(resize_bilinear_k, GRID1(total), dim3(256), 0, ST, x, out, H, W, Ho, Wo, (float)H / (float)Ho,
                     (float)W / (float)Wo, total);
  return wtpse_status();
}
extern "C" int wtpse_relu_mask(const float* dz, const float* ref, float* dy, int accumulate, long long n, void* stream) {
  WTPSE_REQUIRE(dz && ref && dy && n > 0);
  if (n % 4 == 0 && (((uintptr_t)dz | (uintptr_t)ref | (uintptr_t)dy) & 15) == 0)
    hipLaunchKernelGGL(relu_mask_v_k, GRID1(n / 4), dim3(256), 0, ST, reinterpret_cast<const float4*>(dz),
                       reinterpret_cast<const float4*>(ref), reinterpret_cast<float4*>(dy), accumulate, n / 4);
  else
    hipLaunchKernelGGL(relu_mask_k, GRID1(n), dim3(256), 0, ST, dz, ref, dy, accumulate, n);
  return wtpse_status();
}
__global__ __launch_bounds__(256) void copy_w16_k(const float4* __restrict__ src, float4* __restrict__ dst, long long n4) {
  for (long long i = (long long)blockIdx.x * 256 + threadIdx.x; i < n4; i += (long long)gridDim.x * 256) dst[i] = src[i];
}
__global__ __launch_bounds__(256) void copy_w4_k(const float* __restrict__ src, float* __restrict__ dst, long long n) {
  for (long long i = (long long)blockIdx.x * 256 + threadIdx.x; i < n; i += (long long)gridDim.x * 256) dst[i] = src[i];
}
extern "C" int wtpse_copy_probe(const float* src, float* dst, long long n, int bytes_per_lane, void* stream) {
  WTPSE_REQUIRE(src && dst && n > 0 && n % 4 == 0 && (bytes_per_lane == 4 || bytes_per_lane == 16));
  WTPSE_REQUIRE((((uintptr_t)src | (uintptr_t)dst) & 15) == 0);
  if (bytes_per_lane == 16)
    hipLaunchKernelGGL(copy_w16_k, dim3(8192), dim3(256), 0, ST, reinterpret_cast<const float4*>(src), reinterpret_cast<float4*>(dst), n / 4);
  else
    hipLaunchKernelGGL(copy_w4_k, dim3(16384), dim3(256), 0, ST, src, dst, n);
  return wtpse_status();
}
__global__ __launch_bounds__(256) void amax_k(const float* __restrict__ x, long long n, unsigned* __restrict__ table) {
  unsigned m = 0u;
  const long long n4 = n >> 2;
  const uint4* x4 = reinterpret_cast<const uint4*>(x);
  if ((reinterpret_cast<uintptr_t>(x) & 15) == 0) {
    for (long long i = (long long)blockIdx.x * 256 + threadIdx.x; i < n4; i += (long long)gridDim.x * 256) {
      const uint4 v = x4[i];
      m = max(max(m, v.x & 0x7FFFFFFFu), max(v.y & 0x7FFFFFFFu, max(v.z & 0x7FFFFFFFu, v.w & 0x7FFFFFFFu)));
    }
    for (long long i = (n4 << 2) + (long long)blockIdx.x * 256 + threadIdx.x; i < n; i += (long long)gridDim.x * 256)
      m = max(m, __float_as_uint(x[i]) & 0x7FFFFFFFu);
  } else {
    for (long long i = (long long)blockIdx.x * 256 + threadIdx.x; i < n; i += (long long)gridDim.x * 256)
      m = max(m, __float_as_uint(x[i]) & 0x7FFFFFFFu);
  }
  amax_publish_block(table, m, blockIdx.x);
}
extern "C" int wtpse_amax(const float* x, long long n, unsigned* amax_table, void* stream) {
  WTPSE_REQUIRE(amax_table && n >= 0 && (x || n == 0));
  if (hipMemsetAsync(amax_table, 0, AMAX_WORDS * sizeof(unsigned), ST) != hipSuccess) return wtpse_status();
  if (n > 0) {
    const long long blocks = (n / 4 + 255) / 256 + 1;
    hipLaunchKernelGGL(amax_k, dim3((unsigned)(blocks < 2048 ? blocks : 2048)), dim3(256), 0, ST, x, n, amax_table);
  }
  return wtpse_status();
}
extern "C" int wtpse_axpy(float* dst, const float* src, float alpha, long long n, void* stream) {
  WTPSE_REQUIRE(dst && src && n > 0);
  if (n % 4 == 0 && (((uintptr_t)dst | (uintptr_t)src) & 15) == 0)
    hipLaunchKernelGGL(axpy_v_k, GRID1(n / 4), dim3(256), 0, ST, reinterpret_cast<float4*>(dst), reinterpret_cast<const float4*>(src),
                       alpha, n / 4);
  else
    hipLaunchKernelGGL(axpy_k, GRID1(n), dim3(256), 0, ST, dst, src, alpha, n);
  return wtpse_status();
}
extern "C" int wtpse_reduce_rows(const float* partial, int rows, int cols, float* out, int accumulate, float scale, void* stream) {
  WTPSE_REQUIRE(partial && out && rows > 0 && cols > 0);
  if (cols <= 64 && rows >= 1024)
    hipLaunchKernelGGL(reduce_rows_tall_k, dim3(cols), dim3(256), 0, ST, partial, rows, cols, out, accumulate, scale);
  else
    hipLaunchKernelGGL(reduce_rows_k, GRID1(cols), dim3(256), 0, ST, partial, rows, cols, out, accumulate, scale);
  return wtpse_status();
}
extern "C" int wtpse_zero(void* p, long long nbytes, void* stream) {
  WTPSE_REQUIRE(p && nbytes >= 0);
  hipError_t e = hipMemsetAsync(p, 0, (size_t)nbytes, ST);
  return e == hipSuccess ? WTPSE_OK : (int)e;
}
extern "C" int wtpse_attn_fuse_fwd(const float* z, const float* wb, const float* emb, float coef, float* att, float* att_pre,
                                   float* mask, float* fuse, int B, int CE, int HW, void* stream) {
  WTPSE_REQUIRE(z && wb && emb && fuse && B > 0 && CE > 0 && HW > 0);
  long long total = (long long)B * HW;
  hipLaunchKernelGGL(attn_fuse_fwd_k, GRID1(total), dim3(256), 0, ST, z, wb, emb, coef, att, att_pre, mask, fuse, CE, HW, total);
  return wtpse_status();
}
extern "C" int wtpse_attn_fuse_bwd(const float* dfuse, const float* z, const float* emb, const float* att, const float* wb,
                                   float coef, float* demb, float* dz, float* partial, float* d_wb, int accumulate, int B,
                                   int CE, int HW, void* stream) {
  WTPSE_REQUIRE(dfuse && z && emb && att && wb && demb && partial && d_wb && B > 0 && CE > 0 && HW > 0);
  long long total = (long long)B * HW;
  unsigned nb = (unsigned)((total + 255) / 256);
  hipLaunchKernelGGL(attn_fuse_bwd_k, dim3(nb), dim3(256), 0, ST, dfuse, z, emb, att, wb, coef, demb, dz, partial, CE, HW, total);
  if (nb >= 1024)
    hipLaunchKernelGGL(reduce_rows_tall_k, dim3(2), dim3(256), 0, ST, partial, (int)nb, 2, d_wb, accumulate, 1.f);
  else
    hipLaunchKernelGGL(reduce_rows_k, dim3(1), dim3(256), 0, ST, partial, (int)nb, 2, d_wb, accumulate, 1.f);
  return wtpse_status();
}
extern "C" int wtpse_reparam_fwd(const float* mu, const float* logvar, const float* eps, float* z, long long n, void* stream) {
  WTPSE_REQUIRE(mu && logvar && eps && z && n > 0);
  hipLaunchKernelGGL(reparam_fwd_k, GRID1(n), dim3(256), 0, ST, mu, logvar, eps, z, n);
  return wtpse_status();
}
extern "C" int wtpse_reparam_bwd(const float* dz, const float* logvar, const float* eps, float* dlogvar, long long n, void* stream) {
  WTPSE_REQUIRE(dz && logvar && eps && dlogvar && n > 0);
  hipLaunchKernelGGL(reparam_bwd_k, GRID1(n), dim3(256), 0, ST, dz, logvar, eps, dlogvar, n);
  return wtpse_status();
}
extern "C" int wtpse_exp_half(const float* logvar, float* std_, long long n, void* stream) {
  WTPSE_REQUIRE(logvar && std_ && n > 0);
  hipLaunchKernelGGL(exp_half_k, GRID1(n), dim3(256), 0, ST, logvar, std_, n);
  return wtpse_status();
}
extern "C" int wtpse_reparam_student(const float* mu, const float* std_, const float* eps, float* z, long long n, void* stream) {
  WTPSE_REQUIRE(mu && std_ && eps && z && n > 0);
  hipLaunchKernelGGL(reparam_student_k, GRID1(n), dim3(256), 0, ST, mu, std_, eps, z, n);
  return wtpse_status();
}
extern "C" int wtpse_nan_scrub(float* x, long long n, int* flag, void* stream) {
  WTPSE_REQUIRE(x && flag && n > 0);
  hipError_t e = hipMemsetAsync(flag, 0, sizeof(int), ST);
  if (e != hipSuccess) return (int)e;
  hipLaunchKernelGGL(nan_flag_k, GRID1(n), dim3(256), 0, ST, x, n, flag);
  hipLaunchKernelGGL(nan_scrub_k, GRID1(n), dim3(256), 0, ST, x, n, flag);
  return wtpse_status();
}
extern "C" int wtpse_bce_sigmoid_fwd(const float* x, const float* t, long long n, float* partial, float* loss, void* stream) {
  WTPSE_REQUIRE(x && t && partial && loss && n > 0);
  unsigned nb = red_blocks(n);
  hipLaunchKernelGGL(bce_sigmoid_fwd_k, dim3(nb), dim3(256), 0, ST, x, t, n, partial);
  hipLaunchKernelGGL(reduce_rows_k, dim3(1), dim3(256), 0, ST, partial, (int)nb, 1, loss, 0, 1.f / (float)n);
  return wtpse_status();
}
extern "C" int wtpse_bce_sigmoid_bwd(const float* x, const float* t, const float* g, float w, long long n, float* dx, void* stream) {
  WTPSE_REQUIRE(x && t && dx && n > 0);
  hipLaunchKernelGGL(bce_sigmoid_bwd_k, GRID1(n), dim3(256), 0, ST, x, t, g, w, n, dx);
  return wtpse_status();
}
extern "C" int wtpse_pos_weight(const float* mask, const float* t, long long n, float* partial, float* sums, float* pw, void* stream) {
  WTPSE_REQUIRE(mask && t && partial && sums && pw && n > 0);
  unsigned nb = red_blocks(n);
  hipLaunchKernelGGL(sum2_k, dim3(nb), dim3(256), 0, ST, mask, t, n, partial);
  hipLaunchKernelGGL(reduce_rows_k, dim3(1), dim3(256), 0, ST, partial, (int)nb, 2, sums, 0, 1.f);
  hipLaunchKernelGGL(pos_weight_k, dim3(1), dim3(1), 0, ST, sums, pw);
  return wtpse_status();
}
extern "C" int wtpse_pos_weight_from_sums(const float* sums, float* pw, void* stream) {
  WTPSE_REQUIRE(sums && pw);
// ... 92 lines not shown
```

### wt-pse-code_amd/wtpse_hip/csrc/wt_loss.hip

```cpp
#include "common.h"

#define WT_C 16
#define WT_NV 120

template <bool VEC>
__global__ __launch_bounds__(256) void gram_partial_k(const float* __restrict__ z, int HW, int S, int chunk,
                                                      float* __restrict__ partial) {
  __shared__ float red[4 * 256];
  const int tid = threadIdx.x, lane = tid & 63, wave = tid >> 6;
  const int b = blockIdx.x / S, s = blockIdx.x - b * S;
  const int c = lane & 15, q = lane >> 4;
  const int p_begin = s * chunk;
  const int p_end = min(HW, p_begin + chunk);
  const float* row = z + ((size_t)b * WT_C + c) * HW;
  f32x4 acc0 = {0, 0, 0, 0}, acc1 = acc0, acc2 = acc0, acc3 = acc0;
  for (int p0 = p_begin + wave * 64; p0 < p_end; p0 += 512) {
    float v[8][4];
#pragma unroll
    for (int g = 0; g < 8; ++g) {
      int p = p0 + (g >> 2) * 256 + (g & 3) * 16 + q * 4;
      if (VEC) {
        float4 t = make_float4(0.f, 0.f, 0.f, 0.f);
        if (p < p_end) t = *reinterpret_cast<const float4*>(row + p);
        v[g][0] = t.x; v[g][1] = t.y; v[g][2] = t.z; v[g][3] = t.w;
// ... 274 lines not shown
    } else {
      float old = (accumulate & 1) ? db[(size_t)c * HW] : 0.f;
      if ((accumulate & 2) && !(in[c][0] > 0.f)) old = 0.f;
      db[(size_t)c * HW] = old + o[0];
    }
  }
}

static void wt_tail_launch(const float* partial, int S, int B, int HW, float eps, float margin, int domain_num, int per_domain,
                           float* gram, float* v, float* offdiag, float* diag, double* rowval, float* dmmd_dv, float* losses,
                           hipStream_t st) {
  const int R = domain_num * per_domain;
  unsigned* ticket = reinterpret_cast<unsigned*>(rowval + R);
  if (S >= 32)
    hipLaunchKernelGGL(gram_finalize_k<16>, dim3(B), dim3(1024), 0, st, partial, S, HW, eps, gram, v, offdiag, diag, ticket);
  else
    hipLaunchKernelGGL(gram_finalize_k<4>, dim3(B), dim3(256), 0, st, partial, S, HW, eps, gram, v, offdiag, diag, ticket);
  WtFinalArgs fin{offdiag, diag, B, B, margin, losses, ticket};
  hipLaunchKernelGGL(mmd_rows_k, dim3(R), dim3(128), R * sizeof(double), st, v, domain_num, per_domain, rowval, dmmd_dv, fin);
}

extern "C" int wtpse_wt_split(int B, int HW, int* chunk_out) {
  int target = 768 / (B > 0 ? B : 1);
  if (target < 1) target = 1;
  int chunk = ceil_div(ceil_div(HW, target), 512) * 512;
  if (chunk < 2048) chunk = 2048;
  int S = ceil_div(HW, chunk);
  if (chunk_out) *chunk_out = chunk;
  return S;
}

extern "C" int wtpse_wt_loss_fwd(const float* z, int B, int C, int HW, float eps, float margin, int domain_num,
                                 int per_domain, float* partial, float* gram, float* v, float* offdiag, float* diag,
                                 double* rowval, float* dmmd_dv, float* losses, void* stream) {
  WTPSE_REQUIRE(z && partial && gram && v && offdiag && diag && rowval && dmmd_dv && losses);
  WTPSE_REQUIRE(C == WT_C && B > 0 && HW > 1 && domain_num >= 1 && per_domain >= 1);
  const int R = domain_num * per_domain;
  WTPSE_REQUIRE(R <= B);
  hipStream_t st = (hipStream_t)stream;
  int chunk;
  const int S = wtpse_wt_split(B, HW, &chunk);
  const bool vec = (HW % 4 == 0) && (((uintptr_t)z & 15) == 0);
  if (vec)
    hipLaunchKernelGGL(gram_partial_k<true>, dim3(B * S), dim3(256), 0, st, z, HW, S, chunk, partial);
  else
    hipLaunchKernelGGL(gram_partial_k<false>, dim3(B * S), dim3(256), 0, st, z, HW, S, chunk, partial);
  wt_tail_launch(partial, S, B, HW, eps, margin, domain_num, per_domain, gram, v, offdiag, diag, rowval, dmmd_dv, losses, st);
  return wtpse_status();
}

extern "C" int wtpse_wt_loss_fwd_partials(const float* partial, int S, int B, int HW, float eps, float margin, int domain_num,
                                          int per_domain, float* gram, float* v, float* offdiag, float* diag, double* rowval,
                                          float* dmmd_dv, float* losses, void* stream) {
  WTPSE_REQUIRE(partial && gram && v && offdiag && diag && rowval && dmmd_dv && losses);
  WTPSE_REQUIRE(S >= 1 && B > 0 && HW > 1 && domain_num >= 1 && per_domain >= 1);
  const int R = domain_num * per_domain;
  WTPSE_REQUIRE(R <= B);
  hipStream_t st = (hipStream_t)stream;
  wt_tail_launch(partial, S, B, HW, eps, margin, domain_num, per_domain, gram, v, offdiag, diag, rowval, dmmd_dv, losses, st);
  return wtpse_status();
}

extern "C" int wtpse_wt_loss_bwd(const float* z, int B, int C, int HW, float margin, int domain_num, int per_domain,
                                 const float* gram, const float* offdiag, const float* diag, const float* dmmd_dv,
                                 const float* g_off, const float* g_diag, const float* g_dom, float w_off, float w_diag,
                                 float w_dom, float* Mws, float* dz, int accumulate, void* stream) {
  WTPSE_REQUIRE(z && gram && offdiag && diag && dmmd_dv && Mws && dz);
  WTPSE_REQUIRE(C == WT_C && B > 0 && HW > 1);
  const int R = domain_num * per_domain;
  hipStream_t st = (hipStream_t)stream;
  hipLaunchKernelGGL(wt_dgram_k, dim3(B), dim3(256), 0, st, gram, offdiag, diag, dmmd_dv, B, R, HW, margin, g_off, g_diag,
                     g_dom, w_off, w_diag, w_dom, Mws);
  const bool vec = (HW % 4 == 0) && (((uintptr_t)z & 15) == 0) && (((uintptr_t)dz & 15) == 0);
  if (vec) {
    int bpi = ceil_div(HW, 1024);
    hipLaunchKernelGGL(gram_bwd_k<true>, dim3(B * bpi), dim3(256), 0, st, z, Mws, HW, bpi, accumulate, dz);
  } else {
    int bpi = ceil_div(HW, 256);
    hipLaunchKernelGGL(gram_bwd_k<false>, dim3(B * bpi), dim3(256), 0, st, z, Mws, HW, bpi, accumulate, dz);
  }
  return wtpse_status();
}

extern "C" int wtpse_wt_gram_fwd(const float* z, int B, int C, int HW, float eps, float* partial, float* gram, float* v,
                                 float* offdiag, float* diag, void* stream) {
  WTPSE_REQUIRE(z && partial && gram && v && offdiag && diag && C == WT_C && B > 0 && HW > 1);
  hipStream_t st = (hipStream_t)stream;
  int chunk;
  const int S = wtpse_wt_split(B, HW, &chunk);
  const bool vec = (HW % 4 == 0) && (((uintptr_t)z & 15) == 0);
  if (vec)
    hipLaunchKernelGGL(gram_partial_k<true>, dim3(B * S), dim3(256), 0, st, z, HW, S, chunk, partial);
  else
    hipLaunchKernelGGL(gram_partial_k<false>, dim3(B * S), dim3(256), 0, st, z, HW, S, chunk, partial);
  hipLaunchKernelGGL(gram_finalize_k<4>, dim3(B), dim3(256), 0, st, partial, S, HW, eps, gram, v, offdiag, diag, (unsigned*)nullptr);
  return wtpse_status();
}

extern "C" int wtpse_wt_final(const float* offdiag, const float* diag, int B, int Bnorm, float margin, const double* rowval,
                              int R, float* losses, void* stream) {
  WTPSE_REQUIRE(offdiag && diag && rowval && losses && B > 0 && Bnorm >= B && R >= 0);
  hipLaunchKernelGGL(wt_final_k, dim3(1), dim3(256), 0, (hipStream_t)stream, offdiag, diag, B, Bnorm, margin, rowval, R, losses);
  return wtpse_status();
}

extern "C" int wtpse_wt_combine(const float* losses, int nmaps, float den, int mode, float* out, void* stream) {
  WTPSE_REQUIRE(losses && out && nmaps > 0 && den > 0.f);
  hipLaunchKernelGGL(wt_combine_k, dim3(1), dim3(64), 0, (hipStream_t)stream, losses, nmaps, den, mode, out);
  return wtpse_status();
}

extern "C" int wtpse_mmd_fwd(const float* v, int domain_num, int per_domain, double* rowval, float* dmmd_dv, void* stream) {
  WTPSE_REQUIRE(v && rowval && dmmd_dv && domain_num >= 1 && per_domain >= 1);
  const int R = domain_num * per_domain;
  hipLaunchKernelGGL(mmd_rows_k, dim3(R), dim3(128), R * sizeof(double), (hipStream_t)stream, v, domain_num, per_domain,
                     rowval, dmmd_dv, WtFinalArgs{nullptr, nullptr, 0, 0, 0.f, nullptr, nullptr});
  return wtpse_status();
}
```

### wt-pse-code_amd/wtpse_hip/nn.py

```python
import math
import os

import torch
import torch.nn as nn

from . import ops


class ConvP(nn.Module):

    def __init__(self, cin, cout, k):
        super().__init__()
        self.cin, self.cout, self.k = cin, cout, k
        self.weight = nn.Parameter(torch.empty(cout, cin, k, k))
        self.bias = nn.Parameter(torch.empty(cout))
        nn.init.kaiming_uniform_(self.weight, a=math.sqrt(5))
        bound = 1.0 / math.sqrt(cin * k * k)
        nn.init.uniform_(self.bias, -bound, bound)
        self.wf_off = self.wd_off = -1
        self.xf_off = self.xd_off = -1
        self.x16f_off = self.x16d_off = -1


class BNP(nn.Module):
# ... 377 lines not shown
            ops.amax_attach(z, self.amax)
        return z


    @staticmethod
    def parts(a):
        return (a.t, a.pro) if a is not None else (None, None)


def as_act(x):
    return x if isinstance(x, Act) else Act(x)


FWD_AMAX = os.environ.get("WTPSE_FWD_AMAX", "1") != "0"


def act_amax(a):
    if a is None or ops.x3_terms() != 2 or not FWD_AMAX:
        return None
    if a.amax is None:
        raw = ops.amax_of(a.t)
        a.amax = raw if a.pro is None else ops.act_bound(a.pro, raw)
    return a.amax


def _relu_bits(a0, a1):
    return (1 if a0.relu else 0) | (2 if (a1 is not None and a1.relu) else 0)


X3 = os.environ.get("WTPSE_X3", "1") != "0"
X3_WGRAD = os.environ.get("WTPSE_X3_WGRAD", "1") != "0"
WGRAD_R = os.environ.get("WTPSE_WGRAD_R", "1") != "0"
X16 = os.environ.get("WTPSE_X16", "1") != "0" and X3
X16_MIN_K = int(os.environ.get("WTPSE_X16_MIN_K", "8"))


def x3_eligible(k_dim, rows, ksize):
    return X3 and rows > 16 and 16 <= k_dim <= 256 and (ksize == 3 or k_dim >= 64)


def _weights(layer, dgrad=False, wide=False):
    root = layer._root
    x16, x3, w = (layer.x16d_off, layer.xd_off, layer.wd_off) if dgrad else (layer.x16f_off, layer.xf_off, layer.wf_off)
    if x16 >= 0 and not wide:
        return 2, root.x3_ptr(x16)
    if x3 >= 0:
        return 1, root.x3_ptr(x3)
    return 0, root.packed_ptr(w)


def _conv(layer, a0, a1=None, relu_out=False, want_stats=False, want_amax=False):
    a0 = as_act(a0)
    a1 = as_act(a1) if a1 is not None else None
    t1, pro1 = Act.parts(a1)
    out_amax = ops.fwd_amax_table(a0.t.device) if want_amax else None
    layout, wptr = _weights(layer, wide=a1 is not None)
    if layout == 2:
        y, stats, _ = ops.conv16_x3(a0.t, wptr, layer.bias, layer.cout, a0.pro, _relu_bits(a0, None), relu_out, want_stats,
                                    in_amax=act_amax(a0), out_amax=out_amax)
    elif layout == 1:
        y, _, stats = ops.conv_fwd_x3(a0.t, t1, wptr, layer.bias, layer.cout, layer.k, a0.pro, _relu_bits(a0, a1), relu_out, want_stats,
                                      None, None, pro1, act_amax(a0), act_amax(a1), out_amax)
    else:
        y, _, stats = ops.conv_fwd(a0.t, t1, wptr, layer.bias, layer.cout, layer.k, a0.pro, _relu_bits(a0, a1), relu_out, want_stats,
                                   None, None, pro1, out_amax)
    return y, stats


class PreBN:
    __slots__ = ("g", "stats", "coef")

    def __init__(self, g, stats, coef=None):
        self.g, self.stats, self.coef = g, stats, coef


BN_FUSED_STATS = os.environ.get("WTPSE_BN_FUSED_STATS", "1") != "0"
BN_TAIL = os.environ.get("WTPSE_BN_TAIL", "1") != "0"


def _gamax(dy):
    return ops.amax_of(dy) if ops.x3_terms() == 2 else None


def _dgrad(layer, dy, split=None, mask_ref=None, below0=None, below1=None):
    root = layer._root
    below = below0 if below0 is not None else below1
    layout, wptr = _weights(layer, dgrad=True, wide=split is not None)
    if (BN_FUSED_STATS and below is not None and mask_ref is None and below.mean is not None
            and not root.bn_synced and (below1 is None or split is not None)):
        bn = below.bn
        tail = (bn.weight, below.invstd, root.gview(bn.weight), root.gview(bn.bias)) if BN_TAIL else None
        if tail is not None and below.frozen:
            tail += (root.gbias(below.conv),)
        d0, d1, stats, coef = ops.dgrad_bnb(dy, wptr, layout, layer.cin, layer.k, below.y, below.ss, below.mean, below.relu, split,
                                            below1 is not None and below0 is None, tail,
                                            _gamax(dy) if layout == 1 else ops.amax_attached(dy) if layout == 2 else None)
        if below0 is not None:
            return PreBN(d0, stats, coef), d1
        return d0, PreBN(d1, stats, coef)
    if layout == 2:
        return ops.conv16_x3(dy, wptr, None, layer.cin, mask_ref=mask_ref, grad_in=True)[0], None
    if layout == 1:
        return ops.conv_fwd_x3(dy, None, wptr, None, layer.cin, layer.k, None, 0, False, False, split, mask_ref, None, _gamax(dy))[:2]
    return ops.conv_fwd(dy, None, wptr, None, layer.cin, layer.k, None, 0, False, False, split, mask_ref)[:2]


_SIDE = {}
WGRAD_SIDE_STREAM = os.environ.get("WTPSE_WGRAD_STREAM", "1") != "0"


def _side_stream(device, owner=None):
    key = (device, ops.stream_ptr() if owner is None else owner)
    st = _SIDE.get(key)
    if st is None:
        st = _SIDE[key] = torch.cuda.Stream(device=device)
    return st


_SECOND = {}
TEACHER_SIDE_STREAM = os.environ.get("WTPSE_TEACHER_STREAM", "1") != "0"


def second_stream(device):
    if not TEACHER_SIDE_STREAM:
        return None
    key = (device, ops.stream_ptr())
    st = _SECOND.get(key)
    if st is None:
        st = _SECOND[key] = torch.cuda.Stream(device=device)
    return st


def stream_wait(waiter, waited):
    waiter.wait_stream(waited)
    ops.lib().plan_wait(waiter.cuda_stream, waited.cuda_stream)


def note_join(root, stream):
    if all(s is not stream for s in root._join):
        root._join.append(stream)


def _wgrad_side(layer, dy, a0, a1=None):
    root = layer._root
    if root._affine_only:
        return
    if not WGRAD_SIDE_STREAM:
        return _wgrad(layer, dy, a0, a1, with_bias=False)
    a0 = as_act(a0)
    a1 = as_act(a1) if a1 is not None else None
    amax = _gamax(dy)
    kernel, tables = _wgrad_kernel(layer, dy, a0, a1, False)
    main = torch.cuda.current_stream()
    side = _side_stream(dy.device)
    stream_wait(side, main)
    with torch.cuda.stream(side):
        _wgrad_launch(kernel, tables, layer, dy, a0, a1, False)
    for t in (dy, amax, a0.t, a0.pro) + tables[1:] + Act.parts(a1):
        if t is not None:
            t.record_stream(side)
    note_join(root, side)


def _wgrad_kernel(layer, dy, a0, a1, with_bias):
    c0, small = a0.t.shape[1], layer.cin % 32 != 0 and layer.cout % 32 != 0
    if (X3 and X3_WGRAD and WGRAD_R and layer.k == 3 and
            ops.wgrad_r_supported(layer.cin, layer.cout, 3, c0 if a1 is not None else 16, a0.t.shape[3]) and (not with_bias or small)):
        return "r", (ops.amax_attached(dy) if small else _gamax(dy), act_amax(a0), act_amax(a1))
    if X3 and X3_WGRAD and not with_bias and ops.wgrad_x3_supported(layer.cin, layer.cout, layer.k, c0 if a1 is not None else 8):
        return "x3", (None, None, None)
    return "fp32", (None, None, None)


def _wgrad_launch(kernel, tables, layer, dy, a0, a1, with_bias):
    root = layer._root
    t1, pro1 = Act.parts(a1)
    dw = root.gview(layer.weight)
    db = root.gview(layer.bias) if with_bias else None
    if kernel == "r":
        ops.conv_wgrad_r(dy, a0.t, t1, dw, db, a0.pro, _relu_bits(a0, a1), False, pro1, *tables)
    elif kernel == "x3":
        ops.conv_wgrad_x3(dy, a0.t, t1, layer.k, dw, a0.pro, _relu_bits(a0, a1), False, pro1)
    else:
        ops.conv_wgrad(dy, a0.t, t1, layer.k, dw, db, a0.pro, _relu_bits(a0, a1), False, pro1)


def _wgrad(layer, dy, a0, a1=None, with_bias=True):
    if layer._root._affine_only:
        return
    a0 = as_act(a0)
    a1 = as_act(a1) if a1 is not None else None
    kernel, tables = _wgrad_kernel(layer, dy, a0, a1, with_bias)
    _wgrad_launch(kernel, tables, layer, dy, a0, a1, with_bias)


def _blend_state(root, training, want_tape):
    blend = root.bn_blend
    if blend is None or training:
        return None
    if want_tape:
        raise RuntimeError("bn_blend: no backward through blended BatchNorm statistics (call update() outside adapt.blended)")
    if root.bn_synced:
        raise RuntimeError("bn_blend is not supported together with synchronised BatchNorm")
    if ops.lib()._rec is not None:
        raise RuntimeError("bn_blend is eager only: it cannot be recorded into a launch plan")
    return blend


def _bn_coeffs(root, bn, y, stats, training, tab=None, raw_amax=None, want_tape=False, blend=None):
    if blend is not None:
        tab = ops.fwd_amax_table(y.device)
        return blend.finalize(bn, y, stats, tab), None, None, tab
    if not training:
        if want_tape:
            ss, mean, invstd = ops.bn_eval_coeffs_stats(bn.weight, bn.bias, bn.running_mean, bn.running_var)
        else:
            ss, mean, invstd = ops.bn_eval_coeffs(bn.weight, bn.bias, bn.running_mean, bn.running_var), None, None
        return ss, mean, invstd, (ops.act_bound(ss, raw_amax) if raw_amax is not None else None)
    B, _, H, W = y.shape
    count = B * H * W
    if root.bn_synced:
        stats, count = root._dp.sync_bn_stats(stats, count)
    if tab is None:
        tab = ops.fwd_amax_table(y.device)
    return ops.bn_finalize(stats, count, bn.weight, bn.bias, bn.running_mean, bn.running_var, bn.num_batches_tracked,
                           momentum=root.bn_momentum, act_amax=tab) + (tab,)


def convbn_fwd(conv, bn, a0, a1, relu, training, want_tape=True):
    root = conv._root
    a0 = as_act(a0)
    a1 = as_act(a1) if a1 is not None else None
    tab = ops.fwd_amax_table(a0.t.device) if training else None
    blend = _blend_state(root, training, want_tape)
    if training and BN_TAIL and not root.bn_synced:
        layout, wptr = _weights(conv, wide=a1 is not None)
        t1, pro1 = Act.parts(a1)
        y, ss, mean, invstd = ops.conv_fwd_bnf(a0.t, t1, wptr, layout, conv.bias, conv.cout, conv.k, a0.pro, _relu_bits(a0, a1), pro1,
                                               bn.weight, bn.bias, bn.running_mean, bn.running_var, bn.num_batches_tracked,
                                               momentum=root.bn_momentum, in_amax0=act_amax(a0) if layout else None,
# ... 164 lines not shown
        return None
    if len(ls) == 3 and not (ls[2].cin == 8 and 1 <= ls[2].cout <= 4):
        return None
    if any(l.k != 1 for l in ls) or (x.t.shape[2] * x.t.shape[3]) % 32 != 0:
        return None
    root = ls[0]._root
    off = root.param_offset(ls[0].weight)
    for l in ls:
        for prm in (l.weight, l.bias):
            if root.param_offset(prm) != off:
                return None
            off += prm.numel()
    return ls


def head_fwd(seq, x, idxs, want_tape=True):
    t = Tape()
    t.x, t.acts = as_act(x), []
    ls = _head_fusable(seq, idxs, t.x)
    t.fused = ls is not None
    if t.fused:
        w3, b3 = (ls[2].weight, ls[2].bias) if len(ls) == 3 else (None, None)
        out, t.h1, t.h2 = ops.head_fwd(t.x.t, t.x.pro, t.x.relu, ls[0].weight, ls[0].bias, ls[1].weight, ls[1].bias, w3, b3,
                                       want_tape, x_amax=act_amax(t.x))
        return out, t
    h = t.x
    for n, i in enumerate(idxs):
        last = n == len(idxs) - 1
        h, _ = _conv(seq[i], h, None, not last, False)
        t.acts.append(h)
    return h, t


def head_bwd(seq, t, d, idxs):
    if t.fused:
        ls = [seq[i] for i in idxs]
        root = ls[0]._root
        views = [root.gview(prm) for l in ls for prm in (l.weight, l.bias)]
        dparams = root.grange(ls[0].weight, sum(v.numel() for v in views))
        return ops.head_bwd(d, t.x.t, t.x.pro, t.x.relu, t.h1, t.h2, ls[0].weight, ls[1].weight,
                            ls[2].weight if len(ls) == 3 else None, dparams, b1=ls[0].bias, x_amax=act_amax(t.x), dy_amax=_gamax(d))
    for n in reversed(range(len(idxs))):
        layer = seq[idxs[n]]
        inp = t.x if n == 0 else t.acts[n - 1]
        _wgrad(layer, d, inp)
        d, _ = _dgrad(layer, d, mask_ref=(t.acts[n - 1] if n > 0 else None))
    return d


WT_FUSED_GRAM = os.environ.get("WTPSE_WT_FUSED_GRAM", "1") != "0"


def _conv_gram(layer, a0):
    a0 = as_act(a0)
    out_amax = ops.fwd_amax_table(a0.t.device)
    layout, wptr = _weights(layer)
    if layout == 2:
        y, _, g = ops.conv16_x3(a0.t, wptr, layer.bias, 16, a0.pro, _relu_bits(a0, None), False, want_gram=True,
                                in_amax=act_amax(a0), out_amax=out_amax)
        return y, g
    assert layout == 0, "a 16-output-channel layer has no x3 layout"
    return ops.conv_fwd_gram(a0.t, wptr, layer.bias, a0.pro, _relu_bits(a0, None), False, out_amax)


def deepwt_fwd(wt, x, want_tape=True, want_gram=False):
    t = Tape()
    a, b = wt.DoubleConv.double_conv, wt.DoubleConv2.double_conv
    t.x = x
    t.g1 = t.g2 = None
    fused = want_gram and WT_FUSED_GRAM and a[2].cout == 16 and a[2].k == 3 and b[2].cout == 16
    t.h1, _ = _conv(a[0], x, None, True, want_amax=True)
    if fused:
        t.z1, t.g1 = _conv_gram(a[2], t.h1)
    else:
        t.z1, _ = _conv(a[2], t.h1, want_amax=True)
    t.h2, _ = _conv(b[0], Act(t.z1, None, True), None, True, want_amax=True)
    if fused:
        t.z2, t.g2 = _conv_gram(b[2], t.h2)
    else:
        t.z2, _ = _conv(b[2], t.h2, want_amax=True)
    return t


def deepwt_bwd(wt, t, dz2, dz1_extra=None):
    a, b = wt.DoubleConv.double_conv, wt.DoubleConv2.double_conv
    _wgrad(b[2], dz2, t.h2)
    d, _ = _dgrad(b[2], dz2, mask_ref=t.h2)
    _wgrad(b[0], d, Act(t.z1, None, True))
    dz1, _ = _dgrad(b[0], d, mask_ref=t.z1)
    if dz1_extra is not None:
        dz1_extra(dz1)
    _wgrad(a[2], dz1, t.h1)
    d, _ = _dgrad(a[2], dz1, mask_ref=t.h1)
    _wgrad(a[0], d, t.x)


def teacher_fwd(tn, feat, mask, training, want_logvar=True, want_tape=True):
    t = Tape()
    inc = tn.inc.double_conv
    feat = as_act(feat)
    m1, t.i0 = convbn_fwd(inc[0], inc[1], mask, None, True, training, want_tape)
    m2, t.i3 = convbn_fwd(inc[3], inc[4], m1, None, True, training, want_tape)
    t.m2, t.feat = m2, feat
    t.xf, _ = _conv(tn.fusion[0], m2, feat, True, want_amax=True)
    fmap, t.unet = unet_fwd(tn, t.xf, training, want_tape)
    t.mu, t.hmu = head_fwd(tn.mu_prior, fmap, (0, 2, 4), want_tape)
    if want_logvar:
        t.logvar, t.hlv = head_fwd(tn.logvar_prior, fmap, (0, 2, 4), want_tape)
    return t


def teacher_bwd(tn, t, dmu, dlogvar):
    d = head_bwd(tn.mu_prior, t.hmu, dmu, (0, 2, 4))
    if dlogvar is not None:
        d2 = head_bwd(tn.logvar_prior, t.hlv, dlogvar, (0, 2, 4))
        ops.axpy(d, d2)
    dxf = unet_bwd(tn, t.unet, d, mask_x=t.xf)
    _wgrad(tn.fusion[0], dxf, t.m2, t.feat)
    dm2, dfeat = _dgrad(tn.fusion[0], dxf, split=t.m2.t.shape[1], below0=t.i3)
    inc = tn.inc.double_conv
    dm1, _ = convbn_bwd(inc[3], inc[4], t.i3, dm2, below0=t.i0)
    convbn_bwd(inc[0], inc[1], t.i0, dm1, need_dx=False)
    return dfeat
```

### wt-pse-code_amd/wtpse_hip/ops.py

```python
import torch

from .lib import lib

_WS = {}


_RAW_STREAM = getattr(torch._C, "_cuda_getCurrentRawStream", None)


def stream_ptr():
    if _RAW_STREAM is not None:
        return _RAW_STREAM(torch.cuda.current_device())
    return torch.cuda.current_stream().cuda_stream


def ptr(t):
    return 0 if t is None else t.data_ptr()


def _chk(t, name="tensor"):
    if t is None:
        return
    if not (t.is_cuda and t.dtype == torch.float32 and t.is_contiguous()):
        raise ValueError("%s must be a contiguous fp32 tensor in device memory (got %s, %s, contiguous=%s)"
                         % (name, t.device, t.dtype, t.is_contiguous()))


def workspace(tag, nfloats, device):
    key = (str(device), stream_ptr(), tag)
    buf = _WS.get(key)
    if buf is None or buf.numel() < nfloats:
        buf = torch.empty(max(int(nfloats), 1024), dtype=torch.float32, device=device)
        _WS[key] = buf
    return buf


def _out_pair(split, B, cout, H, W, device):
    if split is None:
        return torch.empty((B, cout, H, W), dtype=torch.float32, device=device), None, cout
    csplit = int(split)
    return (torch.empty((B, csplit, H, W), dtype=torch.float32, device=device),
            torch.empty((B, cout - csplit, H, W), dtype=torch.float32, device=device), csplit)


def _stats_blocks(layout, B, H, W, cout=0, ksize=0):
    if layout == 1:
        return lib().query("wtpse_conv_x3_stats_blocks", B, H, W, cout, int(ksize))
    return lib().query("wtpse_conv_stats_blocks", B, H, W)


def _conv_launch(name, layout, in_amax, in0, in1, wpacked_ptr, bias, cout, ksize, pro0, pro_relu, relu_out, want_stats, split, mask_ref,
                 pro1, out_amax):
    _chk(in0, "in0"); _chk(in1, "in1"); _chk(pro0, "pro0"); _chk(pro1, "pro1")
    B, C0, H, W = in0.shape
    C1 = 0 if in1 is None else in1.shape[1]
    out0, out1, csplit = _out_pair(split, B, cout, H, W, in0.device)
    stats = None
    if want_stats:
        stats = torch.empty((_stats_blocks(layout, B, H, W, cout, ksize), cout, 2), dtype=torch.float32, device=in0.device)
    lib().call(name, ptr(in0), C0, ptr(in1), C1, wpacked_ptr, ptr(bias), ptr(pro0), ptr(pro1), int(pro_relu), ptr(out0),
               ptr(out1), csplit, ptr(stats), B, H, W, cout, ksize, int(relu_out), ptr(mask_ref), *in_amax, ptr(out_amax), stream_ptr())
    if out_amax is not None:
        amax_attach(out0, out_amax)
    return out0, out1, stats


def conv_fwd(in0, in1, wpacked_ptr, bias, cout, ksize, pro0=None, pro_relu=0, relu_out=False, want_stats=False,
             split=None, mask_ref=None, pro1=None, out_amax=None):
    return _conv_launch("wtpse_conv_fwd", 0, (), in0, in1, wpacked_ptr, bias, cout, ksize, pro0, pro_relu, relu_out, want_stats, split,
                        mask_ref, pro1, out_amax)


def conv_fwd_gram(in0, wpacked_ptr, bias, pro0=None, pro_relu=0, relu_out=False, out_amax=None):
    _chk(in0, "in0"); _chk(pro0, "pro0")
    B, C0, H, W = in0.shape
    L = lib()
    out = torch.empty((B, 16, H, W), dtype=torch.float32, device=in0.device)
    nblk = _stats_blocks(0, B, H, W)
    partial = torch.empty((nblk, 256), dtype=torch.float32, device=in0.device)
    L.call("wtpse_conv_fwd_gram", ptr(in0), C0, wpacked_ptr, ptr(bias), ptr(pro0), int(pro_relu), ptr(out), ptr(partial), B, H, W,
           16, int(relu_out), ptr(out_amax), stream_ptr())
    if out_amax is not None:
        amax_attach(out, out_amax)
    return out, (partial, nblk // B)


X16_SIZE = 8 + 5 * 3 * 64 * 8 + 5 * 2 * 64 * 8


def conv16_x3(in0, wx16_ptr, bias, cout, pro0=None, pro_relu=0, relu_out=False, want_stats=False, want_gram=False, mask_ref=None,
              bnb=None, grad_in=False, in_amax=None, out_amax=None):
    _chk(in0, "in0"); _chk(pro0, "pro0"); _chk(mask_ref, "mask_ref")
    B, C0, H, W = in0.shape
    L = lib()
    out = torch.empty((B, cout, H, W), dtype=torch.float32, device=in0.device)
    nblk = _stats_blocks(2, B, H, W)
    stats = torch.empty((nblk, cout, 2), dtype=torch.float32, device=in0.device) if (want_stats or bnb is not None) else None
    gram = torch.empty((nblk, 256), dtype=torch.float32, device=in0.device) if want_gram else None
    bn_ss = bn_mean = None
    bn_relu = 0
    if bnb is not None:
        mask_ref, bn_ss, bn_mean, bn_relu = bnb
        _chk(mask_ref, "bn_y"); _chk(bn_ss, "bn_ss"); _chk(bn_mean, "bn_mean")
        assert mask_ref.shape == out.shape
    L.call("wtpse_conv16_x3", ptr(in0), C0, wx16_ptr, ptr(bias), ptr(pro0), int(pro_relu), ptr(out), ptr(stats), ptr(gram),
           ptr(mask_ref), ptr(bn_ss), ptr(bn_mean), int(bool(bn_relu)), B, H, W, cout, int(relu_out), int(bool(grad_in)),
           ptr(amax_attached(in0)) if grad_in else ptr(in_amax), ptr(out_amax), stream_ptr())
    if out_amax is not None:
        amax_attach(out, out_amax)
    return out, stats, ((gram, nblk // B) if want_gram else None)


def x3_packed_size(rows, k, taps):
    return 32 + ((k + 15) & ~15) * ((rows + 31) & ~31) * taps * 3


def x3_terms():
    return lib().query("wtpse_x3_terms", -1)


AMAX_WORDS = 1024
_AMAX = {}
_AMAX_TABLES = 512


class _Arena:
    __slots__ = ("buf", "next", "retired")

    def __init__(self, buf):
        self.buf, self.next, self.retired = buf, 0, []

    def take(self, n):
        off = self.next
        if self.buf is None or off + n > self.buf.numel():
            return None
        self.next = off + n
        return self.buf[off:off + n]

    def renew(self, buf):
        self.retired.append(self.buf)
        del self.retired[:-3]
        self.buf, self.next = buf, 0

    def __getitem__(self, i):
        return (self.buf, self.next)[i]


def amax_begin(device):
    buf = zero_(torch.empty(_AMAX_TABLES * AMAX_WORDS, dtype=torch.int32, device=device))
    st = _AMAX.get(device)
    if st is None:
        _AMAX[device] = _Arena(buf)
    else:
        st.renew(buf)


def _amax_table(device):
    if x3_terms() != 2:
        return None
    st = _AMAX.get(device)
    t = st.take(AMAX_WORDS) if st is not None else None
    return t if t is not None else zero_(torch.empty(AMAX_WORDS, dtype=torch.int32, device=device))


_FWD_SCOPES = []
FWD_SCOPE_TABLES = 256


class fwd_scope(_Arena):
    __slots__ = ()

    def __init__(self, device):
        super().__init__(zero_(torch.empty(FWD_SCOPE_TABLES * AMAX_WORDS, dtype=torch.int32, device=device)) if x3_terms() == 2 else None)

    def __enter__(self):
        _FWD_SCOPES.append(self)
        return self

# ... 311 lines not shown
    coef = workspace("bn_bwd_coef", C * 3, g.device)
    dy = _dy_like(g)
    lib().call("wtpse_bn_bwd_from_stats_frozen", ptr(g), ptr(stats), stats.shape[0], ptr(gamma), ptr(invstd), ptr(coef), ptr(dgamma),
               ptr(dbeta), ptr(dbias), int(accumulate), ptr(dy), B, C, H * W, ptr(dy.wt_amax), stream_ptr())
    return dy


def bn_bwd_finalize_coef_frozen(stats, gamma, invstd, dgamma, dbeta, dbias, accumulate=False):
    _chk(stats, "stats")
    C = stats.shape[1]
    coef = torch.empty((C, 3), dtype=torch.float32, device=stats.device)
    lib().call("wtpse_bn_bwd_finalize_coef_frozen", ptr(stats), stats.shape[0], C, ptr(gamma), ptr(invstd), ptr(coef), ptr(dgamma),
               ptr(dbeta), ptr(dbias), int(accumulate), stream_ptr())
    return coef


def bn_bwd_scale_coef(g, coef):
    _chk(g, "g"); _chk(coef, "coef")
    B, C, H, W = g.shape
    dy = _dy_like(g)
    lib().call("wtpse_bn_bwd_scale_coef", ptr(g), ptr(coef), ptr(dy), B, C, H * W, ptr(dy.wt_amax), stream_ptr())
    return dy


def bn_frozen_fold_spec(g, y, gamma, running_mean, running_var, eps=1e-5):
    r = 1.0 / torch.sqrt(running_var + eps)
    s = gamma * r
    sum_g = g.sum(dim=(0, 2, 3))
    sum_gy = (g * (y - running_mean.view(1, -1, 1, 1))).sum(dim=(0, 2, 3))
    return s.view(1, -1, 1, 1) * g, r * sum_gy, sum_g, s * sum_g, running_mean, r


class WtLossState:
    __slots__ = ("z", "gram", "offdiag", "diag", "dmmd_dv", "losses", "v", "B", "HW", "D", "n", "margin")


def bn_bwd_apply_coef(g, y, coef):
    _chk(g, "g"); _chk(y, "y")
    B, C, H, W = y.shape
    dy = _dy_like(y)
    lib().call("wtpse_bn_bwd_apply_coef", ptr(g), ptr(y), ptr(coef), ptr(dy), B, C, H * W, ptr(dy.wt_amax), stream_ptr())
    return dy


def wt_loss_fwd(z, domain_num, per_domain, margin=0.0, eps=1e-5, losses_out=None, gram_partial=None):
    _chk(z, "z")
    B, C, H, W = z.shape
    HW = H * W
    dev = z.device
    L = lib()
    S = L.query("wtpse_wt_split", B, HW, 0)
    R = domain_num * per_domain
    st = WtLossState()
    partial = workspace("wt_partial", B * S * 256, dev) if gram_partial is None else None
    st.gram = torch.empty((B, 256), dtype=torch.float32, device=dev)
    st.v = torch.empty((B, 120), dtype=torch.float32, device=dev)
    st.offdiag = torch.empty((B,), dtype=torch.float32, device=dev)
    st.diag = torch.empty((B,), dtype=torch.float32, device=dev)
    rowval = torch.empty((max(R, 1) + 1,), dtype=torch.float64, device=dev)
    st.dmmd_dv = torch.empty((max(R, 1), 120), dtype=torch.float32, device=dev)
    st.losses = losses_out if losses_out is not None else torch.empty((3,), dtype=torch.float32, device=dev)
    if gram_partial is not None:
        gp, gs = gram_partial
        assert C == 16 and gp.shape[0] == B * gs
        L.call("wtpse_wt_loss_fwd_partials", ptr(gp), int(gs), B, HW, float(eps), float(margin), int(domain_num), int(per_domain),
               ptr(st.gram), ptr(st.v), ptr(st.offdiag), ptr(st.diag), ptr(rowval), ptr(st.dmmd_dv), ptr(st.losses), stream_ptr())
    else:
        L.call("wtpse_wt_loss_fwd", ptr(z), B, C, HW, float(eps), float(margin), int(domain_num), int(per_domain),
               ptr(partial), ptr(st.gram), ptr(st.v), ptr(st.offdiag), ptr(st.diag), ptr(rowval), ptr(st.dmmd_dv),
               ptr(st.losses), stream_ptr())
    st.z, st.B, st.HW, st.D, st.n, st.margin = z, B, HW, domain_num, per_domain, float(margin)
    return st


def wt_loss_bwd(st, dz, accumulate, g_off=None, g_diag=None, g_dom=None, w_off=1.0, w_diag=1.0, w_dom=1.0):
    _chk(dz, "dz")
    _amax_stale(dz)
    Mws = workspace("wt_M", st.B * 256, dz.device)
    lib().call("wtpse_wt_loss_bwd", ptr(st.z), st.B, 16, st.HW, st.margin, st.D, st.n, ptr(st.gram), ptr(st.offdiag),
               ptr(st.diag), ptr(st.dmmd_dv), ptr(g_off), ptr(g_diag), ptr(g_dom), float(w_off), float(w_diag),
               float(w_dom), ptr(Mws), ptr(dz), int(accumulate), stream_ptr())


def wt_combine(losses, den, mode, out=None):
    if out is None:
        out = torch.empty((4,), dtype=torch.float32, device=losses.device)
    lib().call("wtpse_wt_combine", ptr(losses), losses.shape[0], float(den), int(mode), ptr(out), stream_ptr())
    return out


def maxpool2_fwd(x, pro=None, relu=False):
    _chk(x, "x")
    B, C, H, W = x.shape
    out = torch.empty((B, C, H // 2, W // 2), dtype=torch.float32, device=x.device)
    lib().call("wtpse_maxpool2_fwd", ptr(x), ptr(pro), int(relu), ptr(out), B, C, H, W, stream_ptr())
    return out


def maxpool2_bwd(x, dout, dx, accumulate, pro=None, relu=False, mask=False):
    B, C, H, W = x.shape
    if dx is None:
        dx = torch.empty_like(x)
        accumulate = False
    _amax_stale(dx)
    lib().call("wtpse_maxpool2_bwd", ptr(x), ptr(pro), int(relu), ptr(dout), ptr(dx), int(bool(accumulate)) | (2 if mask else 0),
               B, C, H, W, stream_ptr())
    return dx


def maxpool2_bwd_bnb(x, dout, dx, pro, relu, mean):
    B, C, H, W = x.shape
    if W % 4 or H % 2 or B * C >= 32768 or pro is None:
        return None
    L = lib()
    acc = dx is not None
    if dx is None:
        dx = torch.empty_like(x)
    _amax_stale(dx)
    stats = torch.empty((L.query("wtpse_maxpool2_bwd_stats_blocks", B, H, W), C, 2), dtype=torch.float32, device=x.device)
    L.call("wtpse_maxpool2_bwd_bnb", ptr(x), ptr(pro), int(relu), ptr(dout), ptr(dx), int(acc), ptr(mean), ptr(stats), B, C, H, W,
           stream_ptr())
    return dx, stats


def upsample2x_fwd(x, pro=None, relu=False):
    _chk(x, "x")
    B, C, H, W = x.shape
    out = torch.empty((B, C, 2 * H, 2 * W), dtype=torch.float32, device=x.device)
    lib().call("wtpse_upsample2x_fwd", ptr(x), ptr(pro), int(relu), ptr(out), B, C, H, W, stream_ptr())
    return out


def upsample2x_fwd_stats(x):
    _chk(x, "x")
    B, C, H, W = x.shape
    out = torch.empty((B, C, 2 * H, 2 * W), dtype=torch.float32, device=x.device)
    nblk = lib().query("wtpse_upsample2x_stats_blocks", B, H, W)
    stats = torch.empty((nblk, C, 2), dtype=torch.float32, device=x.device)
    lib().call("wtpse_upsample2x_fwd_stats", ptr(x), ptr(out), ptr(stats), B, C, H, W, stream_ptr())
    return out, stats


def upsample2x_bwd(dout):
    _chk(dout, "dout")
    B, C, Ho, Wo = dout.shape
    dx = torch.empty((B, C, Ho // 2, Wo // 2), dtype=torch.float32, device=dout.device)
    amax_attach(dx, _amax_table(dout.device))
    lib().call("wtpse_upsample2x_bwd", ptr(dout), ptr(dx), 0, B, C, Ho // 2, Wo // 2, ptr(dx.wt_amax), stream_ptr())
    return dx


def upsample2x_bwd_bn(g, bn_y, coef):
    _chk(g, "g"); _chk(bn_y, "bn_y"); _chk(coef, "coef")
    B, C, Ho, Wo = g.shape
    assert bn_y.shape == g.shape and coef.shape == (C, 3) and Wo % 8 == 0, (g.shape, bn_y.shape, coef.shape)
    dx = torch.empty((B, C, Ho // 2, Wo // 2), dtype=torch.float32, device=g.device)
    amax_attach(dx, _amax_table(g.device))
    lib().call("wtpse_upsample2x_bwd_bn", ptr(g), ptr(bn_y), ptr(coef), ptr(dx), B, C, Ho // 2, Wo // 2, ptr(dx.wt_amax), stream_ptr())
    return dx


def resize_bilinear(x, size):
    _chk(x, "x")
    B, C, H, W = x.shape
    Ho, Wo = int(size[0]), int(size[1])
    out = torch.empty((B, C, Ho, Wo), dtype=torch.float32, device=x.device)
    lib().call("wtpse_resize_bilinear", ptr(x), ptr(out), B, C, H, W, Ho, Wo, stream_ptr())
    return out


def relu_mask(dz, ref, out=None, accumulate=False):
    _chk(dz, "dz"); _chk(ref, "ref")
    if out is None:
        out = torch.empty_like(dz)
        accumulate = False
    _amax_stale(out)
    lib().call("wtpse_relu_mask", ptr(dz), ptr(ref), ptr(out), int(accumulate), dz.numel(), stream_ptr())
    return out


def _amax_stale(t):
    if t is not None and getattr(t, "wt_amax", None) is not None:
        t.wt_amax = None


def axpy(dst, src, alpha=1.0):
    _amax_stale(dst)
    lib().call("wtpse_axpy", ptr(dst), ptr(src), float(alpha), dst.numel(), stream_ptr())
    return dst


def zero_(t):
    _amax_stale(t)
    lib().call("wtpse_zero", ptr(t), t.numel() * t.element_size(), stream_ptr())
    return t


def head_fwd(x, pro, relu, w1, b1, w2, b2, w3, b3, want_tape=True, x_amax=None, want_h1=False):
    _chk(x, "x"); _chk(pro, "pro")
    B, C, H, W = x.shape
    three = w3 is not None
    nc = w3.shape[0] if three else 0
    h1 = torch.empty((B, 32, H, W), dtype=torch.float32, device=x.device) if (want_tape and (want_h1 or x3_terms() != 2)) else None
    h2 = torch.empty((B, 8, H, W), dtype=torch.float32, device=x.device) if (want_tape or not three) else None
    y = torch.empty((B, nc, H, W), dtype=torch.float32, device=x.device) if three else None
# ... 699 lines not shown
```

Measured before the change: 811.0.

## Fuse WT loss gradient into conv16 dgrad epilogue and add BN-backward add kernel

The WT loss backward term for z1 is now computed as a per-sample 16x16 coefficient matrix up front, then applied inside the masked 16-channel x3 dgrad epilogue through extra MFMAs. This removes a separate pass that read and wrote dz1. A new add_bnb kernel fuses the teacher head gradient sum with the BN-backward ReLU masking and the per-channel stat partials, replacing an axpy and a later stats pass. An optional side-stream wgrad path for the deep WT block is also added but is off by default. The trade-off is a more complex epilogue and new constraints on when each fused path applies.

```diff
diff --git a/include/wtpse_hip.h b/include/wtpse_hip.h
--- a/include/wtpse_hip.h
+++ b/include/wtpse_hip.h
@@ -31,6 +31,8 @@
                     float* out0, float* stats, float* gram_partial, const float* mask_ref, const float* bn_ss,
                     const float* bn_mean, int bn_relu, int B, int H, int W, int Cout, int relu_out, int in_is_grad,
                     const unsigned* in_amax, unsigned* out_amax, void* stream);
+int wtpse_conv16_x3_wt(const float* dy, int C, const unsigned short* wx16, float* out0, const float* mask_ref, const float* wt_m,
+                       int B, int H, int W, int Cout, const unsigned* in_amax, void* stream);
 int wtpse_pack_conv16_x3(const float* params, const int* desc, int n_desc, unsigned short* packed, void* stream);
 
 int wtpse_dgrad_bnb(const float* dy, int C, const float* wpacked, float* out0, float* out1, int Csplit, const float* bn_y,
@@ -136,6 +138,10 @@
                       const float* gram, const float* offdiag, const float* diag, const float* dmmd_dv,
                       const float* g_off, const float* g_diag, const float* g_dom, float w_off, float w_diag, float w_dom,
                       float* Mws, float* dz, int accumulate, void* stream);
+int wtpse_wt_loss_bwd_coef(const float* z, int B, int C, int HW, float margin, int domain_num, int per_domain,
+                           const float* gram, const float* offdiag, const float* diag, const float* dmmd_dv,
+                           const float* g_off, const float* g_diag, const float* g_dom, float w_off, float w_diag, float w_dom,
+                           float* Mws, float* dz, int accumulate, void* stream);
 int wtpse_wt_combine(const float* losses, int nmaps, float den, int mode, float* out, void* stream);
 int wtpse_mmd_fwd(const float* v, int domain_num, int per_domain, double* rowval, float* dmmd_dv, void* stream);
 
@@ -145,6 +151,9 @@
 int wtpse_maxpool2_bwd_stats_blocks(int B, int H, int W);
 int wtpse_maxpool2_bwd_bnb(const float* x, const float* pro, int relu, const float* dout, float* dx, int accumulate,
                            const float* mean, float* stats, int B, int C, int H, int W, void* stream);
+int wtpse_add_bnb_stats_blocks(int B, int HW);
+int wtpse_add_bnb(const float* a, const float* b, const float* y, const float* ss, int relu, const float* mean, float* g,
+                  float* stats, int B, int C, int HW, void* stream);
 int wtpse_upsample2x_fwd(const float* x, const float* pro, int relu, float* out, int B, int C, int H, int W, void* stream);
 int wtpse_upsample2x_bwd(const float* dout, float* dx, int accumulate, int B, int C, int H, int W, unsigned* amax, void* stream);
 int wtpse_upsample2x_bwd_bn(const float* g, const float* bn_y, const float* bn_coef, float* dx, int B, int C, int H, int W,
diff --git a/wt-pse-code_amd/algorithms.py b/wt-pse-code_amd/algorithms.py
--- a/wt-pse-code_amd/algorithms.py
+++ b/wt-pse-code_amd/algorithms.py
@@ -324,6 +324,9 @@
             return self._dp.wt_loss_bwd(st, dz, acc, **kw)
         return ops.wt_loss_bwd(st, dz, acc, **kw)
 
+    def _wt_loss_bwd_coef(self, st, **kw):
+        return None if self._dp is not None else ops.wt_loss_bwd_coef(st, **kw)
+
     def _backward_update(self, t, d_out, d_ins=None, d_dom=None, w_ins=1.0, w_dom=1.0):
         self.begin_backward()
         if d_out is None:
@@ -356,7 +359,8 @@
                 self.grads_ready(self.prior_dist)
                 dz2 = d_relu_z2
                 self._wt_loss_bwd(t.st2, dz2, mask_in=True, **kw)
-                E.deepwt_bwd(self.wt_model, t.w, dz2, lambda dz1: self._wt_loss_bwd(t.st1, dz1, **kw))
+                E.deepwt_bwd(self.wt_model, t.w, dz2, lambda dz1=None: (self._wt_loss_bwd_coef(t.st1, **kw) if dz1 is None
+                                                                        else self._wt_loss_bwd(t.st1, dz1, **kw)))
 
             second = None if (self._dp is not None and self._dp.exact) else E.second_stream(dz_post.device)
             if second is not None:
diff --git a/wt-pse-code_amd/shape_networks.py b/wt-pse-code_amd/shape_networks.py
--- a/wt-pse-code_amd/shape_networks.py
+++ b/wt-pse-code_amd/shape_networks.py
@@ -146,6 +146,9 @@
             return self._dp.wt_loss_bwd(st, dz, acc, **kw)
         return ops.wt_loss_bwd(st, dz, acc, **kw)
 
+    def _wt_loss_bwd_coef(self, st, **kw):
+        return None if self._dp is not None else ops.wt_loss_bwd_coef(st, **kw)
+
     def _backward_update(self, t, g_kd=None, g_off=None, g_diag=None, g_dom=None, w_kd=1.0, w_off=1.0, w_diag=1.0, w_dom=1.0):
         self.begin_backward()
         c = lambda g: g.contiguous() if g is not None else None
@@ -156,7 +159,7 @@
         dz2 = d_relu_z2
         self._wt_loss_bwd(t.st2, dz2, mask_in=True, g_off=g_off, g_diag=g_diag, g_dom=g_dom, w_off=w_off / 3.0, w_diag=2.0 * w_diag / 3.0,
                           w_dom=w_dom / 3.0)
-        E.deepwt_bwd(self.wt_model, t.w2, dz2,
-                     lambda dz1: self._wt_loss_bwd(t.st1, dz1, g_off=g_off, g_diag=g_diag, g_dom=g_dom, w_off=w_off / 3.0,
-                                                   w_diag=0.0, w_dom=w_dom / 3.0))
+        kw1 = dict(g_off=g_off, g_diag=g_diag, g_dom=g_dom, w_off=w_off / 3.0, w_diag=0.0, w_dom=w_dom / 3.0)
+        E.deepwt_bwd(self.wt_model, t.w2, dz2, lambda dz1=None: (self._wt_loss_bwd_coef(t.st1, **kw1) if dz1 is None
+                                                                 else self._wt_loss_bwd(t.st1, dz1, **kw1)))
         self.end_backward()
diff --git a/wt-pse-code_amd/wtpse_hip/csrc/conv.hip b/wt-pse-code_amd/wtpse_hip/csrc/conv.hip
--- a/wt-pse-code_amd/wtpse_hip/csrc/conv.hip
+++ b/wt-pse-code_amd/wtpse_hip/csrc/conv.hip
@@ -29,6 +29,7 @@
   int relu_out;
   int tiles_x, tiles_y;
   int xcd_tiles;
+  const float* wt_m;
 };
 
 
@@ -44,7 +45,7 @@
 
 template <int KS, int MODE, int TWL, bool DB, int EPI>
 __global__ __launch_bounds__(256, 3) void conv_fwd_k(ConvArgs a) {
-  constexpr bool MASK = EPI == 1, BNB = EPI == 2;
+  constexpr bool MASK = EPI == 1 || EPI == 3, BNB = EPI == 2, WTM = EPI == 3;
   constexpr int TAPS = KS * KS, PAD = KS / 2;
   constexpr int TW = 1 << TWL, TH = 256 / TW;
   constexpr int PITCH = TW + 2 * PAD, ROWS = TH + 2 * PAD;
@@ -55,6 +56,7 @@
   constexpr int XT = MODE == 4 ? 2 : 3;
   constexpr bool P16 = (MODE == 0) || XP;
   static_assert(!XP || KS == 3, "MODE 3 / 4 is the 3x3 path");
+  static_assert(!WTM || XP, "EPI 3 is an epilogue of the 16-channel x3 / x2h path");
   constexpr int MT = P16 ? 1 : MODE;
   constexpr int MB = P16 ? 16 : 32;
   constexpr int CB = MB * MT;
@@ -354,6 +356,8 @@
   const __amdgpu_buffer_rsrc_t rs_m = MASK ? make_rsrc(a.mask + (size_t)b * a.Cout * HW, (unsigned)a.Cout * HW * 4u)
                                       : BNB ? make_rsrc(a.mask + (size_t)b * Cbn * HW, (unsigned)Cbn * HW * 4u) : rs_o0;
   const int clane = P16 ? (lane >> 4) * 4 : (lane >> 5) * 4;
+  f32x4 mfr = {0.f, 0.f, 0.f, 0.f};
+  if constexpr (WTM) mfr = *reinterpret_cast<const f32x4*>(a.wt_m + (size_t)b * 256 + (lane & 15) * 16 + clane);
   unsigned pvo[NT];
 #pragma unroll
   for (int nt = 0; nt < NT; ++nt) pvo[nt] = poff[nt] >= 0 ? (unsigned)(clane * HW + poff[nt]) * 4u : BUF_OOB;
@@ -435,6 +439,17 @@
 #pragma unroll
         for (int nt = 0; nt < NT; ++nt) mk[r][nt] = buf_load(rs_m, bn ? pvo[nt] : BUF_OOB, soff);
       }
+    }
+    if constexpr (WTM) {
+#pragma unroll
+      for (int r = 0; r < NACC; ++r)
+#pragma unroll
+        for (int nt = 0; nt < NT; ++nt)
+          if (!(mk[r][nt] > 0.f)) acc[mt][nt][r] = 0.f;
+#pragma unroll
+      for (int nt = 0; nt < NT; ++nt)
+#pragma unroll
+        for (int i = 0; i < 4; ++i) acc[mt][nt] = mfma16(mfr[i], mk[i][nt], acc[mt][nt]);
     }
     float bmu[NACC];
 #pragma unroll
@@ -454,7 +469,7 @@
 #pragma unroll
       for (int nt = 0; nt < NT; ++nt) {
         float v = acc[mt][nt][r];
-        if (MASK && !(mk[r][nt] > 0.f)) v = 0.f;
+        if (MASK && !WTM && !(mk[r][nt] > 0.f)) v = 0.f;
         if (BNB) {
           if (!bn_relu_live_opaque(mk[r][nt], bsc, bsh)) v = 0.f;
           acc[mt][nt][r] = v;
@@ -591,6 +606,8 @@
                          bn.c1 <= c.Cout && bn.c0 % 16 == 0 && (bn.c1 % 16 == 0 || bn.c1 == c.Cout)));
   WTPSE_REQUIRE(c.C1 == 0 || c.C0 % 16 == 0);
   WTPSE_REQUIRE(!(c.out_amax && (c.mask_ref || bnb)));
+  WTPSE_REQUIRE(!c.wt_m || (layout == CONV_C16 && c.mask_ref && !bnb && c.Cout == 16 && c.ksize == 3 && !c.out1 && !c.bias &&
+                            !c.relu_out && !c.stats && !c.gram && (((uintptr_t)c.wt_m) & 15) == 0));
   WTPSE_REQUIRE(!c.gram || (c.Cout == 16 && !c.relu_out));
   WTPSE_REQUIRE(!t.tickets || (bnb && t.partial2 && t.gamma && t.invstd && t.coef && t.dgamma && t.dbeta));
   WTPSE_REQUIRE(!f.tickets || (!bnb && c.stats && !c.gram && f.partial2 && f.gamma && f.beta && f.scale_shift && f.save_mean &&
@@ -616,8 +633,13 @@
   a.B = c.B; a.H = c.H; a.W = c.W; a.C0 = c.C0; a.C1 = c.C1; a.Cin = c.C0 + c.C1; a.CinP = c16 ? 16 : (a.Cin + 3) & ~3;
   a.Cout = c.Cout; a.CoutP = (c.Cout + 15) & ~15; a.Csplit = c.Csplit; a.pro_relu = c.pro_relu; a.relu_out = c.relu_out;
   a.tiles_x = a.tiles_y = 0;
+  a.wt_m = c.wt_m;
 #define FWD(KS, M, DB) (bnb ? launch_fwd<KS, M, DB, 2>(a, st) : c.mask_ref ? launch_fwd<KS, M, DB, 1>(a, st) : launch_fwd<KS, M, DB, 0>(a, st))
-  if (c16) return (g_x3_terms == 2 && (!c.in_is_grad || c.in_amax0)) ? FWD(3, 4, false) : FWD(3, 3, false);
+  if (c16) {
+    const bool x2h = g_x3_terms == 2 && (!c.in_is_grad || c.in_amax0);
+    if (c.wt_m) return x2h ? launch_fwd<3, 4, false, 3>(a, st) : launch_fwd<3, 3, false, 3>(a, st);
+    return x2h ? FWD(3, 4, false) : FWD(3, 3, false);
+  }
   int mode = c.Cout <= 16 ? 0 : (c.Cout % 64 == 0 ? 2 : 1);
   const int tiles = conv_tiling(c.B, c.H, c.W).tiles;
   if (mode == 2 && tiles * (a.CoutP / 64) < 512) mode = 1;
@@ -667,6 +689,16 @@
   c.stats = stats; c.gram = gram_partial; c.mask_ref = mask_ref; c.in_amax0 = in_amax; c.in_is_grad = in_is_grad; c.out_amax = out_amax;
   c.bn.ss = bn_ss; c.bn.mean = bn_mean; c.bn.relu = bn_relu; c.bn.c1 = Cout;
   c.B = B; c.H = H; c.W = W; c.Cout = Cout; c.ksize = 3; c.relu_out = relu_out;
+  return conv_run(c, CONV_C16, (hipStream_t)stream);
+}
+
+extern "C" int wtpse_conv16_x3_wt(const float* dy, int C, const unsigned short* wx16, float* out0, const float* mask_ref,
+                                  const float* wt_m, int B, int H, int W, int Cout, const unsigned* in_amax, void* stream) {
+  WTPSE_REQUIRE(mask_ref && wt_m);
+  ConvCall c;
+  c.in0 = dy; c.C0 = C; c.w = wx16; c.out0 = out0; c.Csplit = Cout; c.mask_ref = mask_ref; c.wt_m = wt_m; c.in_amax0 = in_amax;
+  c.in_is_grad = 1;
+  c.B = B; c.H = H; c.W = W; c.Cout = Cout; c.ksize = 3;
   return conv_run(c, CONV_C16, (hipStream_t)stream);
 }
 
diff --git a/wt-pse-code_amd/wtpse_hip/csrc/internal.h b/wt-pse-code_amd/wtpse_hip/csrc/internal.h
--- a/wt-pse-code_amd/wtpse_hip/csrc/internal.h
+++ b/wt-pse-code_amd/wtpse_hip/csrc/internal.h
@@ -20,6 +20,7 @@
   float* out0 = nullptr; float* out1 = nullptr; int Csplit = 0;
   float* stats = nullptr;
   const float* mask_ref = nullptr;
+  const float* wt_m = nullptr;
   float* gram = nullptr;
   const unsigned* in_amax0 = nullptr; const unsigned* in_amax1 = nullptr;
   int in_is_grad = 0;
diff --git a/wt-pse-code_amd/wtpse_hip/csrc/pointwise.hip b/wt-pse-code_amd/wtpse_hip/csrc/pointwise.hip
--- a/wt-pse-code_amd/wtpse_hip/csrc/pointwise.hip
+++ b/wt-pse-code_amd/wtpse_hip/csrc/pointwise.hip
@@ -382,6 +382,67 @@
   dst[i] = d;
 }
 
+#define ADD_BNB_CHUNK 2048
+template <bool VEC>
+__global__ __launch_bounds__(256) void add_bnb_k(const float* a, const float* __restrict__ b, const float* __restrict__ y,
+                                                 const float* __restrict__ ss, int relu, const float* __restrict__ mean, float* g,
+                                                 float* __restrict__ stats, int BC, int C, int HW) {
+  __shared__ float sh4[4];
+  const int p0 = blockIdx.x * ADD_BNB_CHUNK;
+  for (int bc = blockIdx.y; bc < BC; bc += gridDim.y) {
+    const int c = bc % C;
+    const float sc = relu ? ss[2 * c] : 0.f, sf = relu ? ss[2 * c + 1] : 1.f, mu = mean[c];
+    const size_t base = (size_t)bc * HW;
+    float s1, s2;
+    if (VEC) {
+      float4 gv[2], yv[2];
+#pragma unroll
+      for (int j = 0; j < 2; ++j) {
+        const int p = p0 + j * (ADD_BNB_CHUNK / 2) + threadIdx.x * 4;
+        gv[j] = yv[j] = make_float4(0.f, 0.f, 0.f, 0.f);
+        if (p < HW) {
+          const float4 av = *reinterpret_cast<const float4*>(a + base + p), bv = *reinterpret_cast<const float4*>(b + base + p);
+          yv[j] = *reinterpret_cast<const float4*>(y + base + p);
+          gv[j] = make_float4(av.x + bv.x, av.y + bv.y, av.z + bv.z, av.w + bv.w);
+          bn_relu_mask4(gv[j], yv[j], sc, sf);
+          *reinterpret_cast<float4*>(g + base + p) = gv[j];
+        }
+      }
+      {
+#pragma clang fp contract(off)
+        s1 = ((gv[0].x + gv[0].y) + (gv[0].z + gv[0].w)) + ((gv[1].x + gv[1].y) + (gv[1].z + gv[1].w));
+        s2 = ((gv[0].x * (yv[0].x - mu) + gv[0].y * (yv[0].y - mu)) + (gv[0].z * (yv[0].z - mu) + gv[0].w * (yv[0].w - mu))) +
+             ((gv[1].x * (yv[1].x - mu) + gv[1].y * (yv[1].y - mu)) + (gv[1].z * (yv[1].z - mu) + gv[1].w * (yv[1].w - mu)));
+      }
+    } else {
+      float gv[8], yv[8];
+#pragma unroll
+      for (int j = 0; j < 8; ++j) {
+        const int p = p0 + j * 256 + threadIdx.x;
+        gv[j] = yv[j] = 0.f;
+        if (p < HW) {
+          yv[j] = y[base + p];
+          gv[j] = bn_relu_live(yv[j], sc, sf) ? a[base + p] + b[base + p] : 0.f;
+          g[base + p] = gv[j];
+        }
+      }
+      {
+#pragma clang fp contract(off)
+        s1 = ((gv[0] + gv[1]) + (gv[2] + gv[3])) + ((gv[4] + gv[5]) + (gv[6] + gv[7]));
+        s2 = ((gv[0] * (yv[0] - mu) + gv[1] * (yv[1] - mu)) + (gv[2] * (yv[2] - mu) + gv[3] * (yv[3] - mu))) +
+             ((gv[4] * (yv[4] - mu) + gv[5] * (yv[5] - mu)) + (gv[6] * (yv[6] - mu) + gv[7] * (yv[7] - mu)));
+      }
+    }
+    s1 = block_sum(s1, sh4);
+    s2 = block_sum(s2, sh4);
+    if (threadIdx.x == 0) {
+      float* dst = stats + (((size_t)(bc / C) * gridDim.x + blockIdx.x) * C + c) * 2;
+      dst[0] = s1;
+      dst[1] = s2;
+    }
+  }
+}
+
 __global__ __launch_bounds__(256) void reduce_rows_k(const float* __restrict__ partial, int rows, int cols,
                                                      float* __restrict__ out, int accumulate, float scale) {
   int j = blockIdx.x * 256 + threadIdx.x;
@@ -850,6 +911,19 @@
     hipLaunchKernelGGL(axpy_k, GRID1(n), dim3(256), 0, ST, dst, src, alpha, n);
   return wtpse_status();
 }
+extern "C" int wtpse_add_bnb_stats_blocks(int B, int HW) { return B * ((HW + ADD_BNB_CHUNK - 1) / ADD_BNB_CHUNK); }
+extern "C" int wtpse_add_bnb(const float* a, const float* b, const float* y, const float* ss, int relu, const float* mean, float* g,
+                             float* stats, int B, int C, int HW, void* stream) {
+  WTPSE_REQUIRE(a && b && y && mean && g && stats && (ss || !relu) && B > 0 && C > 0 && HW > 0);
+  WTPSE_REQUIRE((long long)B * C < 32768);
+  const dim3 grid((unsigned)((HW + ADD_BNB_CHUNK - 1) / ADD_BNB_CHUNK), (unsigned)(B * C));
+  if (HW % 4 == 0 && (((uintptr_t)a | (uintptr_t)b | (uintptr_t)y | (uintptr_t)g) & 15) == 0)
+    hipLaunchKernelGGL(add_bnb_k<true>, grid, dim3(256), 0, ST, a, b, y, ss, relu, mean, g, stats, B * C, C, HW);
+  else
+    hipLaunchKernelGGL(add_bnb_k<false>, grid, dim3(256), 0, ST, a, b, y, ss, relu, mean, g, stats, B * C, C, HW);
+  return wtpse_status();
+}
+
 extern "C" int wtpse_reduce_rows(const float* partial, int rows, int cols, float* out, int accumulate, float scale, void* stream) {
   WTPSE_REQUIRE(partial && out && rows > 0 && cols > 0);
   if (cols <= 64 && rows >= 1024)
diff --git a/wt-pse-code_amd/wtpse_hip/csrc/wt_loss.hip b/wt-pse-code_amd/wtpse_hip/csrc/wt_loss.hip
--- a/wt-pse-code_amd/wtpse_hip/csrc/wt_loss.hip
+++ b/wt-pse-code_amd/wtpse_hip/csrc/wt_loss.hip
@@ -380,6 +380,17 @@
   return wtpse_status();
 }
 
+extern "C" int wtpse_wt_loss_bwd_coef(const float* z, int B, int C, int HW, float margin, int domain_num, int per_domain,
+                                      const float* gram, const float* offdiag, const float* diag, const float* dmmd_dv,
+                                      const float* g_off, const float* g_diag, const float* g_dom, float w_off, float w_diag,
+                                      float w_dom, float* Mws, float* dz, int accumulate, void* stream) {
+  WTPSE_REQUIRE(gram && offdiag && diag && dmmd_dv && Mws);
+  WTPSE_REQUIRE(C == WT_C && B > 0 && HW > 1);
+  hipLaunchKernelGGL(wt_dgram_k, dim3(B), dim3(256), 0, (hipStream_t)stream, gram, offdiag, diag, dmmd_dv, B,
+                     domain_num * per_domain, HW, margin, g_off, g_diag, g_dom, w_off, w_diag, w_dom, Mws);
+  return wtpse_status();
+}
+
 extern "C" int wtpse_wt_gram_fwd(const float* z, int B, int C, int HW, float eps, float* partial, float* gram, float* v,
                                  float* offdiag, float* diag, void* stream) {
   WTPSE_REQUIRE(z && partial && gram && v && offdiag && diag && C == WT_C && B > 0 && HW > 1);
diff --git a/wt-pse-code_amd/wtpse_hip/nn.py b/wt-pse-code_amd/wtpse_hip/nn.py
--- a/wt-pse-code_amd/wtpse_hip/nn.py
+++ b/wt-pse-code_amd/wtpse_hip/nn.py
@@ -483,10 +483,13 @@
     return ops.amax_of(dy) if ops.x3_terms() == 2 else None
 
 
-def _dgrad(layer, dy, split=None, mask_ref=None, below0=None, below1=None):
+def _dgrad(layer, dy, split=None, mask_ref=None, below0=None, below1=None, wt_m=None):
     root = layer._root
     below = below0 if below0 is not None else below1
     layout, wptr = _weights(layer, dgrad=True, wide=split is not None)
+    if wt_m is not None:
+        assert layout == 2 and mask_ref is not None and below is None
+        return ops.conv16_x3(dy, wptr, None, layer.cin, mask_ref=mask_ref, grad_in=True, wt_m=wt_m)[0], None
     if (BN_FUSED_STATS and below is not None and mask_ref is None and below.mean is not None
             and not root.bn_synced and (below1 is None or split is not None)):
         bn = below.bn
@@ -542,21 +545,21 @@
         root._join.append(stream)
 
 
-def _wgrad_side(layer, dy, a0, a1=None):
+def _wgrad_side(layer, dy, a0, a1=None, with_bias=False):
     root = layer._root
     if root._affine_only:
         return
     if not WGRAD_SIDE_STREAM:
-        return _wgrad(layer, dy, a0, a1, with_bias=False)
+        return _wgrad(layer, dy, a0, a1, with_bias=with_bias)
     a0 = as_act(a0)
     a1 = as_act(a1) if a1 is not None else None
-    amax = _gamax(dy)
-    kernel, tables = _wgrad_kernel(layer, dy, a0, a1, False)
+    amax = None if with_bias else _gamax(dy)
+    kernel, tables = _wgrad_kernel(layer, dy, a0, a1, with_bias)
     main = torch.cuda.current_stream()
     side = _side_stream(dy.device)
     stream_wait(side, main)
     with torch.cuda.stream(side):
-        _wgrad_launch(kernel, tables, layer, dy, a0, a1, False)
+        _wgrad_launch(kernel, tables, layer, dy, a0, a1, with_bias)
     for t in (dy, amax, a0.t, a0.pro) + tables[1:] + Act.parts(a1):
         if t is not None:
             t.record_stream(side)
@@ -887,17 +890,25 @@
     return t
 
 
-def deepwt_bwd(wt, t, dz2, dz1_extra=None):
+WT_BWD_FUSED = os.environ.get("WTPSE_WT_BWD_FUSED", "1") != "0"
+WT_WGRAD_SIDE = os.environ.get("WTPSE_WT_WGRAD_STREAM", "0") == "1"
+
+
+def deepwt_bwd(wt, t, dz2, dz1_matrix=None):
     a, b = wt.DoubleConv.double_conv, wt.DoubleConv2.double_conv
-    _wgrad(b[2], dz2, t.h2)
+    wgrad = (lambda l, dy, x: _wgrad_side(l, dy, x, with_bias=True)) if WT_WGRAD_SIDE else _wgrad
+    wt_m = None
+    if WT_BWD_FUSED and dz1_matrix is not None and b[0].cin == 16 and _weights(b[0], dgrad=True)[0] == 2:
+        wt_m = dz1_matrix()
+    wgrad(b[2], dz2, t.h2)
     d, _ = _dgrad(b[2], dz2, mask_ref=t.h2)
-    _wgrad(b[0], d, Act(t.z1, None, True))
-    dz1, _ = _dgrad(b[0], d, mask_ref=t.z1)
-    if dz1_extra is not None:
-        dz1_extra(dz1)
-    _wgrad(a[2], dz1, t.h1)
+    wgrad(b[0], d, Act(t.z1, None, True))
+    dz1, _ = _dgrad(b[0], d, mask_ref=t.z1, wt_m=wt_m)
+    if wt_m is None and dz1_matrix is not None:
+        dz1_matrix(dz1)
+    wgrad(a[2], dz1, t.h1)
     d, _ = _dgrad(a[2], dz1, mask_ref=t.h1)
-    _wgrad(a[0], d, t.x)
+    wgrad(a[0], d, t.x)
 
 
 def teacher_fwd(tn, feat, mask, training, want_logvar=True, want_tape=True):
@@ -915,11 +926,22 @@
     return t
 
 
+ADD_BNB = os.environ.get("WTPSE_ADD_BNB", "1") != "0"
+
+
 def teacher_bwd(tn, t, dmu, dlogvar):
     d = head_bwd(tn.mu_prior, t.hmu, dmu, (0, 2, 4))
     if dlogvar is not None:
         d2 = head_bwd(tn.logvar_prior, t.hlv, dlogvar, (0, 2, 4))
-        ops.axpy(d, d2)
+        last = t.unet.u4.c3
+        r = None
+        if (ADD_BNB and BN_FUSED_STATS and not tn.up4.conv3._root.bn_synced and t.unet.u4.swapped and last.mean is not None
+                and last.relu):
+            r = ops.add_bnb(d, d2, last.y, last.ss, last.relu, last.mean)
+        if r is not None:
+            d = PreBN(*r)
+        else:
+            ops.axpy(d, d2)
     dxf = unet_bwd(tn, t.unet, d, mask_x=t.xf)
     _wgrad(tn.fusion[0], dxf, t.m2, t.feat)
     dm2, dfeat = _dgrad(tn.fusion[0], dxf, split=t.m2.t.shape[1], below0=t.i3)
diff --git a/wt-pse-code_amd/wtpse_hip/ops.py b/wt-pse-code_amd/wtpse_hip/ops.py
--- a/wt-pse-code_amd/wtpse_hip/ops.py
+++ b/wt-pse-code_amd/wtpse_hip/ops.py
@@ -89,11 +89,19 @@
 
 
 def conv16_x3(in0, wx16_ptr, bias, cout, pro0=None, pro_relu=0, relu_out=False, want_stats=False, want_gram=False, mask_ref=None,
-              bnb=None, grad_in=False, in_amax=None, out_amax=None):
+              bnb=None, grad_in=False, in_amax=None, out_amax=None, wt_m=None):
     _chk(in0, "in0"); _chk(pro0, "pro0"); _chk(mask_ref, "mask_ref")
     B, C0, H, W = in0.shape
     L = lib()
     out = torch.empty((B, cout, H, W), dtype=torch.float32, device=in0.device)
+    if wt_m is not None:
+        _chk(wt_m, "wt_m")
+        assert grad_in and mask_ref is not None and cout == 16 and bnb is None and bias is None and pro0 is None and not (
+            relu_out or want_stats or want_gram or out_amax is not None or pro_relu), "wt_m: the plain masked data gradient only"
+        assert mask_ref.shape == out.shape and wt_m.numel() >= B * 256
+        L.call("wtpse_conv16_x3_wt", ptr(in0), C0, wx16_ptr, ptr(out), ptr(mask_ref), ptr(wt_m), B, H, W, cout,
+               ptr(amax_attached(in0)), stream_ptr())
+        return out, None, None
     nblk = _stats_blocks(2, B, H, W)
     stats = torch.empty((nblk, cout, 2), dtype=torch.float32, device=in0.device) if (want_stats or bnb is not None) else None
     gram = torch.empty((nblk, 256), dtype=torch.float32, device=in0.device) if want_gram else None
@@ -571,6 +579,14 @@
                float(w_dom), ptr(Mws), ptr(dz), int(accumulate), stream_ptr())
 
 
+def wt_loss_bwd_coef(st, g_off=None, g_diag=None, g_dom=None, w_off=1.0, w_diag=1.0, w_dom=1.0):
+    M = workspace("wt_M_fused", st.B * 256, st.gram.device)
+    lib().call("wtpse_wt_loss_bwd_coef", 0, st.B, 16, st.HW, st.margin, st.D, st.n, ptr(st.gram), ptr(st.offdiag), ptr(st.diag),
+               ptr(st.dmmd_dv), ptr(g_off), ptr(g_diag), ptr(g_dom), float(w_off), float(w_diag), float(w_dom), ptr(M), 0, 0,
+               stream_ptr())
+    return M
+
+
 def wt_combine(losses, den, mode, out=None):
     if out is None:
         out = torch.empty((4,), dtype=torch.float32, device=losses.device)
@@ -610,6 +626,19 @@
     L.call("wtpse_maxpool2_bwd_bnb", ptr(x), ptr(pro), int(relu), ptr(dout), ptr(dx), int(acc), ptr(mean), ptr(stats), B, C, H, W,
            stream_ptr())
     return dx, stats
+
+
+def add_bnb(a, b, y, ss, relu, mean, out=None):
+    _chk(a, "a"); _chk(b, "b"); _chk(y, "y")
+    B, C, H, W = y.shape
+    if B * C >= 32768 or a.shape != y.shape or b.shape != y.shape:
+        return None
+    L = lib()
+    g = a if out is None else out
+    _amax_stale(g)
+    stats = torch.empty((L.query("wtpse_add_bnb_stats_blocks", B, H * W), C, 2), dtype=torch.float32, device=y.device)
+    L.call("wtpse_add_bnb", ptr(a), ptr(b), ptr(y), ptr(ss), int(bool(relu)), ptr(mean), ptr(g), ptr(stats), B, C, H * W, stream_ptr())
+    return g, stats
 
 
 def upsample2x_fwd(x, pro=None, relu=False):
```

After: 819.9, median of 6. 1.1% higher.
